# cvjena/ITAL

Measured on AMD Instinct MI355X. Metric: MI-scored candidates/sec per fetch_unlabelled(k) round, higher is better.
Workload: dtype f64; 1 GPU; USPS-shaped synthetic 9298x256, k=4, perfect user, full 2^t enumeration, fetch_unlabelled + update per step; n=9298, d=256, k=4, parallelism=candidate rows sharded over 1 GPU(s), 1 record all-gather per greedy step

## Files before the change

include/ital_hip.h:

```cpp
#ifndef ITAL_HIP_H
#define ITAL_HIP_H

#include <stdint.h>

#ifdef __cplusplus
extern "C" {
#endif

typedef struct ihipStream_t* hipStream_t;

#define ITAL_MAX_T 8
#define ITAL_REC_HEADER 10
#define ITAL_JUMP_BITS 48
#define ITAL_GENERIC_MAX_DIM 20
#define ITAL_GENERIC_MAX_REL 16
#define ITAL_GENERIC_MAX_CALLS (1 << 22)
#define ITAL_TOPK_MAX 4096
#define ITAL_ROUND_MAX_CAND (1 << 21)

const char* ital_version(void);
const char* ital_last_error(void);
int64_t ital_launch_count(void);


int ital_row_norms(const double* X, int64_t n, int ldx, double* xnorm, hipStream_t stream);

int ital_rbf_cols(const double* X, const double* xnorm, int64_t n, int ldx, const double* Xs, const double* sn,
                  int c, double var, double length_scale, double* out, int64_t ldo, hipStream_t stream);

int ital_cross_cov_cols(const double* X, const double* xnorm, int64_t n, int ldx, const double* Xs,
                        const double* sn, int c, const double* W, int ldw, const double* V, int64_t ldv, int m,
                        double var, double length_scale, double* out, int64_t ldo, hipStream_t stream);

int ital_chol_append(const double* XT, const double* XTn, int ldx, double* L, int ldl, double* alpha,
                     const double* ynew, int m, int c, double var, double length_scale, double noise, int* status,
                     hipStream_t stream);

typedef struct ital_label_batch {
    int c;
    int slot[16];
    double y[16];
} ital_label_batch;
int ital_stage_labelled(const double* rows, int ldx, ital_label_batch lb, double* XT_dst, double* XTn_dst, double* y_dst,
                        hipStream_t stream);

typedef struct ital_append_desc {
    const double* rows;
    int ldx;
    ital_label_batch lb;
    const double* X;
    const double* xnorm;
    int64_t n;
    double* XT;
    double* XTn;
    double* L;
    int ldl;
    double* alpha;
    double* ybuf;
    double* V;
    int64_t ldv;
    int m;
    double var, length_scale, noise;
    double* mu;
    double* s2;
    int* status;
} ital_append_desc;
int ital_gp_append(const ital_append_desc* a, hipStream_t stream);

int ital_whiten_append(const double* X, const double* xnorm, int64_t n, int ldx, const double* Xnew,
                       const double* snew, int c, const double* L21, int ldw, const double* L22,
                       const double* alpha_new, double* V, int64_t ldv, int m, double var, double length_scale,
                       double* mu, double* s2, hipStream_t stream);

int ital_predict(const double* Xt, int64_t nt, int ldx, const double* XT, const double* XTn, int m, const double* L,
                 int ldl, const double* alpha, double var, double length_scale, double* mean, double* pvar, double* xtn,
                 double* Vt, int64_t ldvt, int clamp, hipStream_t stream);

int ital_topk(const double* v, int64_t n, int64_t index_offset, int k, double* out_vals, int64_t* out_idx, void* work,
              hipStream_t stream);
int64_t ital_topk_workspace(void);

int ital_mvn_seed(int state[6]);
int ital_mvn_draws_per_call(int n);
int ital_mvn_advance(int state[6], int64_t n_draws);
int ital_mvn_round_seeds(int state[6], int64_t n_cand, int k, int seeds[][6]);
int ital_mvn_tables(int t, long long* jump, long long* jumppat, double* vk);
int ital_mvn_generic_tables(int nmax, long long* jump1, double* vk_all);

typedef struct ital_np_legacy_state {
    uint32_t key[624];
    int32_t pos;
    int32_t has_gauss;
    double gauss;
} ital_np_legacy_state;
int ital_np_legacy_normals(ital_np_legacy_state* st, int64_t n_skip, double* out, int64_t n_out, int threads);

typedef struct ital_batch {
    int kmax;
    int ldx;
    int ldw;
    int64_t* bidx;
    int64_t* bgpos;
    int32_t* bsort;
    double* bmu;
    double* sig;
    double* XB;
    double* XBn;
    double* VB;
} ital_batch;

typedef struct ital_score_desc {
    int t;
    int64_t n_cand;
    const int32_t* cand;
    const uint8_t* alive;
    const double* mu;
    const double* s2;
    const double* C;
    int64_t ldc;
    int64_t row_offset;
    int64_t pos_offset;
    const int64_t* gpos;
    ital_batch batch;
    double noise, eps;
    int label_mode;
    double* mi;
    int seed[6];
    const long long* jump;
    const long long* jumppat;
    const double* vk;
    int* status;
    double* work;
    int64_t work_doubles;
    void* ev_start;
    void* ev_stop;
    const double* sel_X;
    const double* sel_xnorm;
    int sel_ldx;
    const double* sel_V;
    int64_t sel_ldv;
    int sel_m, sel_ldw;
    int sel_rank;
    double* sel_record;
    int64_t* sel_ret;
    double* sel_parts;
    int64_t sel_parts_len;
    unsigned int* sel_counter;
} ital_score_desc;

int ital_score_step(const ital_score_desc* d, hipStream_t stream);

int64_t ital_score_workspace(int t, int64_t n_cand);

int ital_record_len(int ldx, int ldw, int kmax);
int64_t ital_round_workspace(int k, int64_t n_cand, int64_t cap_doubles);
int64_t ital_sel_parts_len(int k, int64_t n_cand, int64_t work_doubles);

typedef struct ital_round_desc {
    int k;
    ital_score_desc step;
    int seeds[ITAL_MAX_T + 1][6];
    const long long* jump[ITAL_MAX_T + 1];
    const long long* jumppat[ITAL_MAX_T + 1];
    const double* vk[ITAL_MAX_T + 1];
    void* ev_start[ITAL_MAX_T + 1];
    void* ev_stop[ITAL_MAX_T + 1];
    int64_t n_rows;
    double var, length_scale;
    double* mi_keep;
    int begin;
    const int32_t* cand_prev;
    int64_t n_prev;
    int world;
    double* records_all;
    void* nccl_comm;
    int (*exchange)(void* ctx, const double* record, double* records_all, int rec_len, hipStream_t stream);
    void* exchange_ctx;
} ital_round_desc;
int ital_fetch_round(const ital_round_desc* r, hipStream_t stream);

int ital_select_local(const double* mi, const int32_t* cand, const uint8_t* alive, int64_t n_cand, int64_t pos_offset,
                      const int64_t* gpos, int64_t row_offset, int rank, int mode, const double* mu, const double* s2,
                      const double* X, const double* xnorm, int ldx, const double* V, int64_t ldv, int m, int ldw,
                      const double* C, int64_t ldc, int nprev, int kmax, const int* status, double* work, double* record,
                      hipStream_t stream);

int ital_select_resolve(const double* records, int world, int rec_len, int rank, int mode, int slot,
                        ital_batch batch, uint8_t* alive, int64_t* ret, hipStream_t stream);

int ital_select_exchange(const double* record, double* records_all, int rec_len, void* nccl_comm, hipStream_t stream);

int ital_exchange_info(void* nccl_comm, int* world, int* rank, char* how, int how_len);

int ital_exchange_error(void* nccl_comm, int* async_error);

int ital_select_fused(const double* mi, const int32_t* cand, uint8_t* alive, int64_t n_cand, int64_t pos_offset,
                      const int64_t* gpos, int64_t row_offset, int rank, int mode, const double* mu, const double* s2,
                      const double* X, const double* xnorm, int ldx, const double* V, int64_t ldv, int m, int ldw,
                      const double* C, int64_t ldc, int nprev, int slot, ital_batch batch, const int* status,
                      double* record, int64_t* ret, hipStream_t stream);


int ital_gather_block(const int64_t* cand, int64_t nc, int64_t row0, int64_t n_rows, const double* X, const double* xnorm,
                      int ldx, const double* V, int64_t ldv, int m, const double* mu, const double* s2, double* Xc,
                      double* Vc, int64_t ldc, double* xnc, double* muc, double* s2c, hipStream_t stream);

int ital_cov_block(const double* Xa, const double* an, int64_t na, const double* Xb, const double* bn, int64_t nb,
                   int ldx, const double* Va, int64_t ldva, const double* Vb, int64_t ldvb, int m, double var,
                   double length_scale, double* out, int64_t ldo, hipStream_t stream);

int ital_cov_abs_rowsum(const double* Xa, const double* an, int64_t na, const double* Xb, const double* bn, int64_t nb,
                        int ldx, const double* Va, int64_t ldva, const double* Vb, int64_t ldvb, int m, double var,
                        double length_scale, double* work, int64_t work_len, int accumulate, double* out,
                        hipStream_t stream);

typedef struct ital_mcmi_desc {
    int t;
    int64_t n_i;
    int64_t pos_offset;
    int64_t n_all;
    const uint8_t* alive;
    const double* mu;
    const double* s2;
    const double* cov;
    int64_t ld_cov;
    const double* C;
    int64_t ldc;
    ital_batch batch;
    double noise, eps;
    double* ce;
    double* work;
    int64_t work_doubles;
} ital_mcmi_desc;

int ital_mcmi_score_step(const ital_mcmi_desc* d, hipStream_t stream);
int64_t ital_mcmi_workspace(int t, int64_t n_i);

typedef struct ital_mcmi_round_desc {
    int k;
    ital_mcmi_desc step;
    const double* Xc;
    const double* xnc;
    int ldx;
    const double* Vc;
    int64_t ldv;
    int m, ldw;
    double var, length_scale;
    const int32_t* pos;
    const int* status;
    double* record;
    int64_t* ret;
    int begin;
} ital_mcmi_round_desc;
int ital_mcmi_round(const ital_mcmi_round_desc* r, hipStream_t stream);

typedef struct ital_gscore_desc {
    int64_t n_cand;
    const int32_t* cand;
    const uint8_t* alive;
    const double* mu;
    const double* s2;
    const double* C;
    int64_t ldc;
    int64_t row_offset, pos_offset;
    const int64_t* gpos;
    int nE;
    const int64_t* E_idx;
    const int32_t* E_sort;
    const double* E_mu;
    const double* E_sig;
    int ldE;
    int n_picks;
    const int32_t* pick_pos;
    int subset_mode;
    int fb_mode;
    double label_prob, mistake_prob;
    int label_mode;
    double noise, eps;
    double clip_cov;
    int seed[6];
    const long long* jump1;
    const double* vk;
    int64_t draws_out;
    int64_t draws_in;
    int n_in;
    const int64_t* in_pos;
    int n_dead;
    const int64_t* dead_pos;
    int mc_rel;
    const uint32_t* rel_samples;
    int mc_fb;
    const uint32_t* fb_samples;
    const int64_t* draw_off;
    int64_t* draw_count;
    double* mi;
    int* status;
    double* work;
    int64_t work_doubles;
    unsigned long long* pair_count;
    int defer_join;
} ital_gscore_desc;

int ital_score_generic(const ital_gscore_desc* d, hipStream_t stream);
int64_t ital_score_generic_workspace(const ital_gscore_desc* d);
int ital_score_generic_join(hipStream_t stream);

typedef struct ital_ctx ital_ctx;
int ital_ctx_create(int64_t n_total, int d, double length_scale, double var, double noise, int capacity, int rank, int world,
                    void* nccl_comm, ital_ctx** out);
int ital_ctx_destroy(ital_ctx* ctx);
int ital_ctx_fit(ital_ctx* ctx, const double* rows, int on_device, hipStream_t stream);
int ital_ctx_update(ital_ctx* ctx, const int64_t* idx, const double* y, int c, hipStream_t stream);
int ital_ctx_fetch(ital_ctx* ctx, int k, int64_t* picks, hipStream_t stream);
int ital_ctx_predict_stored(ital_ctx* ctx, double* mean, double* variance, hipStream_t stream);
int64_t ital_ctx_local_rows(const ital_ctx* ctx, int64_t* row0);

#ifdef __cplusplus
}
#endif
#endif
```

ital_amd/_fast_round.py:

```python
import collections
import ctypes
import time

import numpy as np
import torch

from . import _lib, mvn_stream, sharding
from ._batch import (Scored, ensure_step_buffers, fill_score_desc, fill_score_select, lattice_label, lattice_tables)
from ._lib import check
from .gp import _ptr, _stream
from .retrieval_base import UnseenList

PREPARED, COMPACT, UPLOAD = "prepared", "compact", "upload"

DeviceList = collections.namedtuple("DeviceList", "buffers unseen version picks n_loc")


class Prepared(collections.namedtuple("Prepared", "desc slot k n n_loc m begin cur state_before state_after draws events sig")):
    __slots__ = ()

    def matches(self, k, n, m, stream_state, signature):
        return (self.k == k and self.n == n and self.m == m and self.state_before == tuple(stream_state)
                and self.sig == signature)

    def patch_share(self, n_loc, pos_offset):
        d = self.desc.step
        d.n_cand, d.pos_offset = n_loc, pos_offset
        return self._replace(n_loc=n_loc, events=[ev[:2] + (n_loc,) + ev[3:] for ev in self.events])


def plan_round(candidates, buffers, record, prepared, keep_scores, k, n, m, stream_state, signature):
    follows = (isinstance(candidates, UnseenList) and record is not None and record.buffers is buffers
               and record.unseen is candidates and record.version == candidates.version - 1
               and tuple(sorted(record.picks)) == candidates.last_removed)
    if not follows:
        return UPLOAD
    if prepared is not None and not keep_scores and prepared.matches(k, n, m, stream_state, signature):
        return PREPARED
    return COMPACT


class RoundBuffers(object):

    def __init__(self, learner, b):
        self.L, self.b = learner, b
        self.lists, self.cur = None, 0
        self.descs = None
        self.next = None
        self.exchange_cb = None
        self.exchange_exc = None
        self.device_list = None

    def invalidate(self):
        self.device_list = None

    def drop_prepared(self):
        if self.next is not None:
            for ev in self.next.events:
                self.L.event_pool += [ev[3], ev[4]]
            self.next = None

    def ensure(self, n_loc, k):
        L, b = self.L, self.b
        dev = L.gp.device
        grown = ensure_step_buffers(b, n_loc, L._sel_parts_doubles(k, n_loc), dev)
        if grown or self.lists is None or self.lists[0].numel() < n_loc:
            self.lists = [torch.empty(max(n_loc, 1), dtype=torch.int32, device=dev) for _ in range(2)]
            self.cur = 0
            self.descs = [_lib.ItalRoundDesc(), _lib.ItalRoundDesc()]
            self.drop_prepared()
            self.invalidate()

    def host_exchange(self):
        if self.exchange_cb is None:
            b, group = self.b, self.L.gp.group

            def exchange(ctx, record, records_all, rec_len, stream):
                try:
                    sharding.gather_records(b["rec"], b["rec_all"], group)
                    return 0
                except Exception as e:
                    self.exchange_exc = e
                    return -5
            self.exchange_cb = _lib.EXCHANGE_FN(exchange)
        return self.exchange_cb

    def signature(self, k):
        L, b = self.L, self.b
        gp = L.gp
        w = b.get("qmc_work")
        return (id(b), k, gp.cap, gp.ldv, gp.V.data_ptr(), gp.mu.data_ptr(), 0 if w is None else w.data_ptr(),
                float(L.noise), float(L.eps), float(L.var), float(L.length_scale), L.label_estimation, L.qmc_work_bytes,
                L.profile is not None, repr(L.profile_steps))

    def prepare(self, slot, k, n, m, begin, cur, state_before, *, n_prev=0, n_loc=None, pos_offset=0):
        L, b = self.L, self.b
        gp = L.gp
        r = self.descs[slot]
        d = r.step
        r.k, r.n_rows, r.var, r.length_scale = k, gp.n, float(L.var), float(L.length_scale)
        r.begin, r.cand_prev, r.n_prev = begin, (_ptr(self.lists[cur ^ 1]) if begin == 2 else None), (n_prev if begin == 2 else 0)
        n_loc = n if n_loc is None else n_loc
        fill_score_desc(d, gp, b, Scored(b["mi"], self.lists[cur], b["alive"], n_loc, pos_offset, None, gp.row0), L._user())
        r.world, r.records_all, r.nccl_comm, r.exchange = 0, None, None, _lib.EXCHANGE_FN(0)
        if gp.collective:
            kind, comm = L._round_transport()
            r.world, r.records_all = gp.world, _ptr(b["rec_all"])
            if kind == "nccl":
                r.nccl_comm = comm
            else:
                r.exchange = self.host_exchange()
        fill_score_select(d, gp, b, m, b["ret"])
        r.mi_keep = None
        work = None
        if k >= 3:
            work = L._qmc_workspace(b, k, n_loc)
            d.work, d.work_doubles = _ptr(work), work.numel()
        events = self._lattice_steps(r, k, n, n_loc, work)
        st6 = (ctypes.c_int * 6)(*state_before)
        check(_lib.lib().ital_mvn_round_seeds(st6, n, k, ctypes.byref(r.seeds)))
        draws = sum(mvn_stream.step_draws(t, n - (t - 1)) for t in range(3, k + 1))
        return Prepared(r, slot, k, n, n_loc, m, begin, cur, tuple(state_before), tuple(int(v) for v in st6), draws, events,
                        self.signature(k))

    def _lattice_steps(self, r, k, n, n_loc, work):
        L, b = self.L, self.b
        gp = L.gp
        events = []
        for t in range(1, k + 1):
            r.ev_start[t] = r.ev_stop[t] = None
            if t >= 3:
                r.jump[t], r.jumppat[t], r.vk[t] = [_ptr(x) for x in lattice_tables(b, t, gp.device)]
                if L.profile is not None and (L.profile_steps is None or t in L.profile_steps):
                    k0, k1 = L._event(), L._event()
                    r.ev_start[t], r.ev_stop[t] = k0.cuda_event, k1.cuda_event
                    events.append((lattice_label(work, t, n_loc), t,
                                   n - (t - 1) if not gp.collective else n_loc, k0, k1))
        return events


class FastRound(object):
    def __init__(self, learner, k, candidates):
        self.t_enter = time.perf_counter()
        self.L, self.k, self.candidates, self.gp = learner, k, candidates, learner.gp
        self.n = len(candidates)
        self.listed = isinstance(candidates, UnseenList)
        self.stream = mvn_stream.GLOBAL
        self.lo = self.n_loc = self.rb = self.p = self.keep = self.t_call = None

    def run(self):
        L = self.L
        self._share()
        self._buffers()
        self.p = p = self._descriptor()
        L.last_round = (p.begin, p.slot)
        self._keep_scores()
        saved_stream = (self.stream.state, self.stream.draws)
        self._stamp_call()
        self._call()
        self.stream.state, self.stream.draws = p.state_after, self.stream.draws + p.draws
        if L.profile is not None:
            L.profile += p.events
        self._prepare_next()
        ret, status = self._download()
        return self._finish(ret, status, saved_stream)

    def _share(self):
        gp, c = self.gp, self.candidates
        lo, hi = (c.count_below(gp.row0), c.count_below(gp.row1)) if gp.collective else (0, self.n)
        self.lo, self.n_loc = lo, hi - lo

    def _buffers(self):
        L = self.L
        b = L._buffers(self.k)
        if L._round_bufs is None:
            L._round_bufs = RoundBuffers(L, b)
        self.rb = L._round_bufs
        self.rb.ensure(self.n_loc, self.k)

    def _descriptor(self):
        L, gp, rb, k, n, n_loc = self.L, self.gp, self.rb, self.k, self.n, self.n_loc
        dl, p = rb.device_list, rb.next
        plan = plan_round(self.candidates, rb, dl, p, L.keep_scores, k, n, gp.m, self.stream.state,
                          rb.signature(k) if p is not None else None)
        rb.invalidate()
        if plan == PREPARED:
            rb.next = None
            rb.cur = p.cur
            return p.patch_share(n_loc, self.lo) if gp.collective else p
        rb.drop_prepared()
        if plan == COMPACT:
            begin, n_prev = 2, dl.n_loc
            rb.cur ^= 1
        else:
            begin, n_prev = 1, 0
            c = self.candidates
            share = c.in_rows(gp.row0, gp.row1) if self.listed else np.asarray(c, dtype=np.int64)
            rb.lists[rb.cur][:n_loc].copy_(torch.from_numpy((share - gp.row0).astype(np.int32)))
        return rb.prepare(0, k, n, gp.m, begin, rb.cur, self.stream.state, n_prev=n_prev, n_loc=n_loc, pos_offset=self.lo)

    def _keep_scores(self):
        if self.L.keep_scores:
            self.keep = torch.zeros((self.k, self.n_loc), dtype=torch.float64, device=self.gp.device)
            self.p.desc.mi_keep = _ptr(self.keep)

    def _stamp_call(self):
        hc = self.L.host_clock
        if hc is not None:
            self.t_call = t_call = time.perf_counter()
            if hc.get("t_download") is not None:
                hc["gap_s"] += t_call - hc["t_download"]
                hc["gaps"] += 1
                hc["prologue_s"] = hc.get("prologue_s", 0.0) + (t_call - self.t_enter)

    def _call(self):
        rb = self.rb
        rc = _lib.lib().ital_fetch_round(ctypes.byref(self.p.desc), _stream())
        if rc and rb.exchange_exc is not None:
            exc, rb.exchange_exc = rb.exchange_exc, None
            raise exc
        check(rc)

    def _prepare_next(self):
        L, gp, rb, p, k, n, n_loc = self.L, self.gp, self.rb, self.p, self.k, self.n, self.n_loc
        if n - k >= k and gp.m + k <= gp.cap and not L.keep_scores:
            rb.next = rb.prepare(p.slot ^ 1, k, n - k, gp.m + k, 2, rb.cur ^ 1, self.stream.state, n_prev=n_loc,
                                 n_loc=n_loc if gp.collective else n - k, pos_offset=self.lo)

    def _download(self):
        L, k, hc = self.L, self.k, self.L.host_clock
        if hc is not None:
            hc["enqueue_s"] += time.perf_counter() - self.t_call
        host = L._download(self.rb.b["ret"], "the picks of the round", L._step_estimate_s(k, self.n_loc)).tolist()
        if hc is not None:
            hc["t_download"] = time.perf_counter()
        keep = self.keep
        L.last_scores = [keep[t, :self.n_loc] for t in range(k)] if keep is not None else []
        return host[:k], host[self.rb.b["kmax"]]

    def _finish(self, ret, status, saved_stream):
        L, gp, c = self.L, self.gp, self.candidates
        if status & 8:
            raise RuntimeError("ital_amd: the candidate list kept on the device lost track of the host's (internal error)")
        if status & 6:
            gp.status.bitwise_and_(~6)
            self.stream.state, self.stream.draws = saved_stream
            return L._fetch_generic(self.k, c.array() if self.listed else c)
        if status:
            gp.check_status(status)
        ret = [int(i) for i in ret]
        L._last_batch = (self.rb.b, list(ret))
        if self.listed:
            self.rb.device_list = DeviceList(self.rb, c, c.version, ret, self.n_loc)
        return ret
```

ital_amd/_lib.py:

```python
import ctypes
import os

HERE = os.path.dirname(os.path.abspath(__file__))
LIB_PATH = os.environ.get("ITAL_HIP_LIB", os.path.join(HERE, "libital_hip.so"))

c_void_p, c_int, c_int64, c_double = ctypes.c_void_p, ctypes.c_int, ctypes.c_int64, ctypes.c_double

ITAL_MAX_T = 8
ITAL_REC_HEADER = 10
ITAL_JUMP_BITS = 48
ITAL_GENERIC_MAX_DIM = 20
ITAL_GENERIC_MAX_REL = 16
ITAL_GENERIC_MAX_CALLS = 1 << 22
ITAL_TOPK_MAX = 4096
ITAL_ROUND_MAX_CAND = 1 << 21


class ItalBatch(ctypes.Structure):
    _fields_ = [("kmax", c_int), ("ldx", c_int), ("ldw", c_int), ("bidx", c_void_p), ("bgpos", c_void_p),
                ("bsort", c_void_p), ("bmu", c_void_p), ("sig", c_void_p), ("XB", c_void_p), ("XBn", c_void_p),
                ("VB", c_void_p)]


class ItalLabelBatch(ctypes.Structure):
    _fields_ = [("c", c_int), ("slot", c_int * 16), ("y", c_double * 16)]


class ItalAppendDesc(ctypes.Structure):
    _fields_ = [("rows", c_void_p), ("ldx", c_int), ("lb", ItalLabelBatch), ("X", c_void_p), ("xnorm", c_void_p), ("n", c_int64),
                ("XT", c_void_p), ("XTn", c_void_p), ("L", c_void_p), ("ldl", c_int), ("alpha", c_void_p), ("ybuf", c_void_p),
                ("V", c_void_p), ("ldv", c_int64), ("m", c_int), ("var", c_double), ("length_scale", c_double),
                ("noise", c_double), ("mu", c_void_p), ("s2", c_void_p), ("status", c_void_p)]


class ItalScoreDesc(ctypes.Structure):
    _fields_ = [("t", c_int), ("n_cand", c_int64), ("cand", c_void_p), ("alive", c_void_p), ("mu", c_void_p),
                ("s2", c_void_p), ("C", c_void_p), ("ldc", c_int64), ("row_offset", c_int64),
                ("pos_offset", c_int64), ("gpos", c_void_p), ("batch", ItalBatch), ("noise", c_double), ("eps", c_double),
                ("label_mode", c_int), ("mi", c_void_p), ("seed", c_int * 6), ("jump", c_void_p), ("jumppat", c_void_p),
                ("vk", c_void_p), ("status", c_void_p), ("work", c_void_p), ("work_doubles", c_int64), ("ev_start", c_void_p),
                ("ev_stop", c_void_p), ("sel_X", c_void_p), ("sel_xnorm", c_void_p), ("sel_ldx", c_int), ("sel_V", c_void_p),
                ("sel_ldv", c_int64), ("sel_m", c_int), ("sel_ldw", c_int), ("sel_rank", c_int), ("sel_record", c_void_p),
                ("sel_ret", c_void_p), ("sel_parts", c_void_p), ("sel_parts_len", c_int64), ("sel_counter", c_void_p)]


EXCHANGE_FN = ctypes.CFUNCTYPE(c_int, c_void_p, c_void_p, c_void_p, c_int, c_void_p)


class ItalRoundDesc(ctypes.Structure):
    _fields_ = [("k", c_int), ("step", ItalScoreDesc), ("seeds", (c_int * 6) * (ITAL_MAX_T + 1)),
                ("jump", c_void_p * (ITAL_MAX_T + 1)), ("jumppat", c_void_p * (ITAL_MAX_T + 1)),
                ("vk", c_void_p * (ITAL_MAX_T + 1)), ("ev_start", c_void_p * (ITAL_MAX_T + 1)),
                ("ev_stop", c_void_p * (ITAL_MAX_T + 1)), ("n_rows", c_int64), ("var", c_double), ("length_scale", c_double),
                ("mi_keep", c_void_p), ("begin", c_int), ("cand_prev", c_void_p), ("n_prev", c_int64),
                ("world", c_int), ("records_all", c_void_p), ("nccl_comm", c_void_p), ("exchange", EXCHANGE_FN),
                ("exchange_ctx", c_void_p)]


class ItalGscoreDesc(ctypes.Structure):
    _fields_ = [("n_cand", c_int64), ("cand", c_void_p), ("alive", c_void_p), ("mu", c_void_p), ("s2", c_void_p),
                ("C", c_void_p), ("ldc", c_int64), ("row_offset", c_int64), ("pos_offset", c_int64), ("gpos", c_void_p),
                ("nE", c_int), ("E_idx", c_void_p), ("E_sort", c_void_p), ("E_mu", c_void_p), ("E_sig", c_void_p),
                ("ldE", c_int), ("n_picks", c_int), ("pick_pos", c_void_p), ("subset_mode", c_int), ("fb_mode", c_int),
                ("label_prob", c_double), ("mistake_prob", c_double), ("label_mode", c_int), ("noise", c_double),
                ("eps", c_double), ("clip_cov", c_double), ("seed", c_int * 6), ("jump1", c_void_p), ("vk", c_void_p),
                ("draws_out", c_int64), ("draws_in", c_int64), ("n_in", c_int), ("in_pos", c_void_p),
                ("n_dead", c_int), ("dead_pos", c_void_p), ("mc_rel", c_int), ("rel_samples", c_void_p),
                ("mc_fb", c_int), ("fb_samples", c_void_p), ("draw_off", c_void_p), ("draw_count", c_void_p), ("mi", c_void_p),
                ("status", c_void_p), ("work", c_void_p), ("work_doubles", c_int64), ("pair_count", c_void_p),
                ("defer_join", c_int)]


class ItalMcmiDesc(ctypes.Structure):
    _fields_ = [("t", c_int), ("n_i", c_int64), ("pos_offset", c_int64), ("n_all", c_int64), ("alive", c_void_p),
                ("mu", c_void_p), ("s2", c_void_p), ("cov", c_void_p), ("ld_cov", c_int64), ("C", c_void_p),
                ("ldc", c_int64), ("batch", ItalBatch), ("noise", c_double), ("eps", c_double), ("ce", c_void_p),
                ("work", c_void_p), ("work_doubles", c_int64)]


class ItalMcmiRoundDesc(ctypes.Structure):
    _fields_ = [("k", c_int), ("step", ItalMcmiDesc), ("Xc", c_void_p), ("xnc", c_void_p), ("ldx", c_int), ("Vc", c_void_p),
                ("ldv", c_int64), ("m", c_int), ("ldw", c_int), ("var", c_double), ("length_scale", c_double),
                ("pos", c_void_p), ("status", c_void_p), ("record", c_void_p), ("ret", c_void_p), ("begin", c_int)]


class ItalNpLegacyState(ctypes.Structure):
    _fields_ = [("key", ctypes.c_uint32 * 624), ("pos", ctypes.c_int32), ("has_gauss", ctypes.c_int32), ("gauss", c_double)]


SIGNATURES = {
    "ital_version": (ctypes.c_char_p, []),
    "ital_mvn_seed": (c_int, [ctypes.POINTER(c_int)]),
    "ital_mvn_draws_per_call": (c_int, [c_int]),
    "ital_mvn_advance": (c_int, [ctypes.POINTER(c_int), c_int64]),
    "ital_mvn_round_seeds": (c_int, [ctypes.POINTER(c_int), c_int64, c_int, c_void_p]),
    "ital_mvn_tables": (c_int, [c_int, c_void_p, c_void_p, c_void_p]),
    "ital_mvn_generic_tables": (c_int, [c_int, c_void_p, c_void_p]),
    "ital_np_legacy_normals": (c_int, [ctypes.POINTER(ItalNpLegacyState), c_int64, c_void_p, c_int64, c_int]),
    "ital_last_error": (ctypes.c_char_p, []),
    "ital_launch_count": (c_int64, []),
    "ital_row_norms": (c_int, [c_void_p, c_int64, c_int, c_void_p, c_void_p]),
    "ital_rbf_cols": (c_int, [c_void_p, c_void_p, c_int64, c_int, c_void_p, c_void_p, c_int, c_double, c_double,
                              c_void_p, c_int64, c_void_p]),
    "ital_cross_cov_cols": (c_int, [c_void_p, c_void_p, c_int64, c_int, c_void_p, c_void_p, c_int, c_void_p, c_int,
                                    c_void_p, c_int64, c_int, c_double, c_double, c_void_p, c_int64, c_void_p]),
    "ital_chol_append": (c_int, [c_void_p, c_void_p, c_int, c_void_p, c_int, c_void_p, c_void_p, c_int, c_int,
                                 c_double, c_double, c_double, c_void_p, c_void_p]),
    "ital_whiten_append": (c_int, [c_void_p, c_void_p, c_int64, c_int, c_void_p, c_void_p, c_int, c_void_p, c_int,
                                   c_void_p, c_void_p, c_void_p, c_int64, c_int, c_double, c_double, c_void_p,
                                   c_void_p, c_void_p]),
    "ital_stage_labelled": (c_int, [c_void_p, c_int, ItalLabelBatch, c_void_p, c_void_p, c_void_p, c_void_p]),
    "ital_gp_append": (c_int, [ctypes.POINTER(ItalAppendDesc), c_void_p]),
    "ital_predict": (c_int, [c_void_p, c_int64, c_int, c_void_p, c_void_p, c_int, c_void_p, c_int, c_void_p,
                             c_double, c_double, c_void_p, c_void_p, c_void_p, c_void_p, c_int64, c_int, c_void_p]),
    "ital_topk": (c_int, [c_void_p, c_int64, c_int64, c_int, c_void_p, c_void_p, c_void_p, c_void_p]),
    "ital_topk_workspace": (c_int64, []),
    "ital_score_step": (c_int, [ctypes.POINTER(ItalScoreDesc), c_void_p]),
    "ital_score_workspace": (c_int64, [c_int, c_int64]),
    "ital_fetch_round": (c_int, [ctypes.POINTER(ItalRoundDesc), c_void_p]),
    "ital_cov_block": (c_int, [c_void_p, c_void_p, c_int64, c_void_p, c_void_p, c_int64, c_int, c_void_p, c_int64,
                               c_void_p, c_int64, c_int, c_double, c_double, c_void_p, c_int64, c_void_p]),
    "ital_cov_abs_rowsum": (c_int, [c_void_p, c_void_p, c_int64, c_void_p, c_void_p, c_int64, c_int, c_void_p, c_int64,
                                    c_void_p, c_int64, c_int, c_double, c_double, c_void_p, c_int64, c_int, c_void_p,
                                    c_void_p]),
    "ital_mcmi_score_step": (c_int, [ctypes.POINTER(ItalMcmiDesc), c_void_p]),
    "ital_mcmi_workspace": (c_int64, [c_int, c_int64]),
    "ital_score_generic": (c_int, [ctypes.POINTER(ItalGscoreDesc), c_void_p]),
    "ital_score_generic_workspace": (c_int64, [ctypes.POINTER(ItalGscoreDesc)]),
    "ital_select_local": (c_int, [c_void_p, c_void_p, c_void_p, c_int64, c_int64, c_void_p, c_int64, c_int, c_int, c_void_p,
                                  c_void_p, c_void_p, c_void_p, c_int, c_void_p, c_int64, c_int, c_int, c_void_p,
                                  c_int64, c_int, c_int, c_void_p, c_void_p, c_void_p, c_void_p]),
    "ital_select_fused": (c_int, [c_void_p, c_void_p, c_void_p, c_int64, c_int64, c_void_p, c_int64, c_int, c_int, c_void_p,
                                  c_void_p, c_void_p, c_void_p, c_int, c_void_p, c_int64, c_int, c_int, c_void_p,
                                  c_int64, c_int, c_int, ItalBatch, c_void_p, c_void_p, c_void_p, c_void_p]),
    "ital_select_exchange": (c_int, [c_void_p, c_void_p, c_int, c_void_p, c_void_p]),
    "ital_exchange_info": (c_int, [c_void_p, c_void_p, c_void_p, ctypes.c_char_p, c_int]),
    "ital_exchange_error": (c_int, [c_void_p, c_void_p]),
    "ital_score_generic_join": (c_int, [c_void_p]),
    "ital_ctx_create": (c_int, [c_int64, c_int, c_double, c_double, c_double, c_int, c_int, c_int, c_void_p, c_void_p]),
    "ital_ctx_destroy": (c_int, [c_void_p]),
    "ital_ctx_fit": (c_int, [c_void_p, c_void_p, c_int, c_void_p]),
    "ital_ctx_update": (c_int, [c_void_p, c_void_p, c_void_p, c_int, c_void_p]),
    "ital_ctx_fetch": (c_int, [c_void_p, c_int, c_void_p, c_void_p]),
    "ital_ctx_predict_stored": (c_int, [c_void_p, c_void_p, c_void_p, c_void_p]),
    "ital_ctx_local_rows": (c_int64, [c_void_p, c_void_p]),
    "ital_record_len": (c_int, [c_int, c_int, c_int]),
    "ital_round_workspace": (c_int64, [c_int, c_int64, c_int64]),
    "ital_sel_parts_len": (c_int64, [c_int, c_int64, c_int64]),
    "ital_mcmi_round": (c_int, [ctypes.POINTER(ItalMcmiRoundDesc), c_void_p]),
    "ital_gather_block": (c_int, [c_void_p, c_int64, c_int64, c_int64, c_void_p, c_void_p, c_int, c_void_p, c_int64, c_int,
                                  c_void_p, c_void_p, c_void_p, c_void_p, c_int64, c_void_p, c_void_p, c_void_p, c_void_p]),
    "ital_select_resolve": (c_int, [c_void_p, c_int, c_int, c_int, c_int, c_int, ItalBatch, c_void_p, c_void_p,
                                    c_void_p]),
}


class ItalCtxModel(ctypes.Structure):
    _fields_ = [("label_prob", c_double), ("mistake_prob", c_double), ("label_estimation", c_int),
                ("monte_carlo_num_rel", c_int), ("monte_carlo_num_fb", c_int), ("clip_cov", c_double)]


CTX_SIGNATURES = {
    "ital_ctx_set_model": (c_int, [c_void_p, ctypes.POINTER(ItalCtxModel)]),
    "ital_ctx_fetch_list": (c_int, [c_void_p, c_int, c_void_p, c_int64, c_void_p, c_int, c_void_p, c_void_p]),
    "ital_ctx_mcmi_fetch": (c_int, [c_void_p, c_int, c_void_p, c_int64, c_void_p, c_void_p]),
    "ital_ctx_top_results": (c_int, [c_void_p, c_int, c_void_p, c_void_p]),
    "ital_ctx_predict": (c_int, [c_void_p, c_void_p, c_int64, c_void_p, c_void_p, c_void_p]),
    "ital_ctx_revoke": (c_int, [c_void_p, c_void_p, c_int, c_void_p]),
}


DENSE_SIGNATURES = {
    "ital_gram_rows": (c_int, [c_void_p, c_void_p, c_int, c_void_p, c_void_p, c_void_p, c_void_p, c_int, c_int, c_double,
                               c_double, c_double, c_void_p]),
    "ital_chol_batched": (c_int, [c_void_p, c_void_p, c_void_p, c_int, c_int, c_void_p, c_void_p, c_void_p]),
    "ital_chol_solve_batched": (c_int, [c_void_p, c_void_p, c_void_p, c_void_p, c_int, c_void_p, c_void_p]),
    "ital_kernel_matvec": (c_int, [c_void_p, c_void_p, c_int64, c_void_p, c_void_p, c_int64, c_int, c_void_p, c_int64, c_int,
                                   c_double, c_double, c_void_p, c_int64, c_void_p, c_int64, c_void_p]),
    "ital_kernel_matvec_workspace": (c_int64, [c_int64, c_int64]),
}


ADAPT_SIGNATURES = {
    "ital_chol_inv_diag": (c_int, [c_void_p, c_int, c_int64, c_void_p, c_void_p, c_int64, c_void_p, c_void_p]),
    "ital_chol_inv_diag_workspace": (c_int64, [c_int]),
    "ital_adapt_scores": (c_int, [c_void_p, c_void_p, c_void_p, c_int64, c_double, c_void_p, c_void_p, c_void_p]),
    "ital_adapt_error": (c_int, [c_void_p, c_int64, c_void_p, c_int, c_int64, c_void_p, c_void_p, c_double, c_void_p,
                                 c_void_p, c_void_p]),
}


class ItalRemoveDesc(ctypes.Structure):
    _fields_ = [("XT", c_void_p), ("XTn", c_void_p), ("ldx", c_int), ("L", c_void_p), ("ldl", c_int), ("alpha", c_void_p),
                ("V", c_void_p), ("ldv", c_int64), ("n", c_int64), ("mu", c_void_p), ("s2", c_void_p), ("m", c_int), ("p", c_int),
                ("work", c_void_p), ("work_doubles", c_int64), ("status", c_void_p)]


REVOKE_SIGNATURES = {
    "ital_gp_remove": (c_int, [ctypes.POINTER(ItalRemoveDesc), c_void_p]),
    "ital_gp_remove_workspace": (c_int64, [c_int]),
}


class ItalRewhitenDesc(ctypes.Structure):
    _fields_ = [("X", c_void_p), ("n_rows", c_int64), ("ldx", c_int), ("XT", c_void_p), ("XTn", c_void_p), ("L", c_void_p),
                ("ldl", c_int), ("alpha", c_void_p), ("m", c_int), ("var", c_double), ("length_scale", c_double),
                ("xnorm", c_void_p), ("V", c_void_p), ("ldv", c_int64), ("v_rows", c_int), ("mu", c_void_p), ("s2", c_void_p),
                ("chunk", c_int)]


REWHITEN_SIGNATURES = {
    "ital_whiten_rows": (c_int, [ctypes.POINTER(ItalRewhitenDesc), c_void_p]),
    "ital_whiten_rows_chunk": (c_int, []),
}


class ItalEvidenceDesc(ctypes.Structure):
    _fields_ = [("XT", c_void_p), ("XTn", c_void_p), ("ldx", c_int), ("y", c_void_p), ("m", c_int), ("params", c_void_p),
                ("G", c_int), ("K", c_void_p), ("ld", c_int64), ("scores", c_void_p), ("info", c_void_p),
                ("loo_mean", c_void_p), ("loo_var", c_void_p), ("ldm", c_int64), ("status", c_void_p), ("work", c_void_p),
                ("work_doubles", c_int64), ("ev", c_void_p)]


EVIDENCE_SIGNATURES = {
    "ital_gram_grid": (c_int, [c_void_p, c_void_p, c_int, c_int, c_void_p, c_int, c_void_p, c_int64, c_void_p]),
    "ital_chol_inv_diag_batched": (c_int, [c_void_p, c_void_p, c_int, c_int, c_void_p, c_void_p, c_int64, c_void_p, c_int64,
                                           c_void_p]),
    "ital_chol_inv_diag_batched_workspace": (c_int64, [c_int, c_int]),
    "ital_gp_evidence": (c_int, [ctypes.POINTER(ItalEvidenceDesc), c_void_p]),
    "ital_gp_evidence_workspace": (c_int64, [c_int, c_int]),
}


class ItalHipError(RuntimeError):
    pass


def load(path=LIB_PATH):
    if not os.path.exists(path):
        raise ImportError(
            f"{path} not found: build it with `python -m ital_amd.build` (hipcc, gfx950). "
            "ital_amd has no CPU fallback.")
    try:
        import torch
    except ImportError:
        pass
    lib = ctypes.CDLL(path)
    for name, (res, args) in list(SIGNATURES.items()) + list(CTX_SIGNATURES.items()) + list(DENSE_SIGNATURES.items()) + \
            list(ADAPT_SIGNATURES.items()) + list(REVOKE_SIGNATURES.items()) + list(REWHITEN_SIGNATURES.items()) + \
            list(EVIDENCE_SIGNATURES.items()):
        fn = getattr(lib, name)
        fn.restype = res
        fn.argtypes = args
    return lib


_lib = None


def lib():
    global _lib
    if _lib is None:
        _lib = load()
    return _lib


def check(rc):
    if rc != 0:
        raise ItalHipError(f"libital_hip: error {rc}: {lib().ital_last_error().decode()}")


def legacy_normals(n_skip, n_out, threads=1):
    import numpy as np
    n_skip, n_out = int(n_skip), int(n_out)
    state = np.random.get_state(legacy=True)
    if state[0] != "MT19937":
        if n_skip:
            np.random.standard_normal(n_skip)
        return np.random.standard_normal(n_out)
    st = ItalNpLegacyState()
    key = np.ascontiguousarray(state[1], dtype=np.uint32)
    ctypes.memmove(st.key, key.ctypes.data, 624 * 4)
    st.pos, st.has_gauss, st.gauss = int(state[2]), int(state[3]), float(state[4])
    out = np.empty(n_out, dtype=np.float64)
    check(lib().ital_np_legacy_normals(ctypes.byref(st), n_skip, out.ctypes.data, n_out, int(threads)))
    np.random.set_state(("MT19937", np.frombuffer(st.key, dtype=np.uint32).copy(), int(st.pos), int(st.has_gauss),
                         float(st.gauss)))
    return out
```

ital_amd/csrc/chol.hip:

```cpp
#include <hip/hip_runtime.h>
#include <stdint.h>

#include "device_math.h"
#include "ital_hip.h"
#include "ital_internal.h"

namespace ital {

__device__ __forceinline__ double readlane_f64(double v, int l) {
    return __hiloint2double(__builtin_amdgcn_readlane(__double2hiint(v), l), __builtin_amdgcn_readlane(__double2loint(v), l));
}

struct StageArgs {
    const double* rows;
    ital_label_batch lb;
    double* XT_w;
    double* XTn_w;
    double* y_w;
};

__global__ __launch_bounds__(1024) void chol_append_kernel(const double* XT, const double* XTn,
                                                           int ldx, double* __restrict__ L, int ldl,
                                                           double* __restrict__ alpha, const double* ynew,
                                                           int m, int c, double var, double s, double noise,
                                                           int* __restrict__ status, StageArgs sa) {
    __shared__ double S[16][17];
    __shared__ double tvec[16];
    __shared__ double Lb[64][65];
    const int lane = threadIdx.x & 63;
    const int j = threadIdx.x >> 6;
    const int g = m + j;
    double* Lg = L + (int64_t)g * ldl;
    if (sa.rows) {
        if (j < c) {
            const double* src = sa.rows + (int64_t)sa.lb.slot[j] * ldx;
            double* dst = sa.XT_w + (int64_t)j * ldx;
            double acc = 0;
            for (int k = lane; k < ldx; k += 64) {
                const double v = src[k];
                dst[k] = v;
                acc += v * v;
            }
            acc = wave_sum(acc);
            if (lane == 0) { sa.XTn_w[j] = acc; sa.y_w[j] = sa.lb.y[j]; }
        }
        __threadfence_block();
        __syncthreads();
    }
#ifdef ITAL_CHOL_TIMING
    long long tstamp[6];
    tstamp[0] = __builtin_readcyclecounter();
#define CHOL_STAMP(i) tstamp[i] = __builtin_readcyclecounter()
#else
#define CHOL_STAMP(i)
#endif
    {
        const int sub = threadIdx.x & 15;
        const int npair = (m + c) * c;
        for (int p0 = 0; p0 < npair; p0 += (int)blockDim.x >> 4) {
            const int pr = p0 + ((int)threadIdx.x >> 4);
            const bool live = pr < npair;
            const int jn = live ? pr % c : 0, r = live ? pr / c : 0;
            const int gn = m + jn;
            const bool need = live && r <= gn;
            double d0 = 0, d1 = 0;
            if (need) {
                const double* xa = XT + (int64_t)gn * ldx + 2 * sub;
                const double* xb = XT + (int64_t)r * ldx + 2 * sub;
                for (int k0 = 0; k0 < ldx; k0 += 256) {
                    double2 a[8], b[8];
#pragma unroll
                    for (int u = 0; u < 8; u++) {
                        const int k = k0 + 32 * u;
                        const bool in = k + 2 * sub < ldx;
                        a[u] = in ? *reinterpret_cast<const double2*>(xa + k) : double2{0, 0};
                        b[u] = in ? *reinterpret_cast<const double2*>(xb + k) : double2{0, 0};
                    }
#pragma unroll
                    for (int u = 0; u < 8; u++) {
                        d0 = fma(a[u].x, b[u].x, d0);
                        d1 = fma(a[u].y, b[u].y, d1);
                    }
                }
            }
            double dot = d0 + d1;
#pragma unroll
            for (int off = 1; off < 16; off <<= 1) dot += __shfl_xor(dot, off, 64);
            if (need && sub == 0) {
                double kv = var * exp((XTn[gn] + XTn[r] - 2 * dot) / s);
                if (r == gn) kv += noise;
                L[(int64_t)gn * ldl + r] = kv;
            }
        }
    }
    CHOL_STAMP(1);
    for (int r0 = 0; r0 < m; r0 += 64) {
        const int nb = m - r0 < 64 ? m - r0 : 64;
        __syncthreads();
        for (int idx = threadIdx.x; idx < nb * nb; idx += blockDim.x) {
            const int i = idx / nb, q = idx - i * nb;
            Lb[i][q] = L[(int64_t)(r0 + i) * ldl + r0 + q];
        }
        __syncthreads();
        if (j < c) {
            const bool in = lane < nb;
            double b = 0.0;
            if (in) {
                b = Lg[r0 + lane];
                const double* Li = L + (int64_t)(r0 + lane) * ldl;
                for (int q = 0; q < r0; q++) b = fma(-Li[q], Lg[q], b);
            }
            const double dinv = in ? 1.0 / Lb[lane][lane] : 1.0;
            double lq = Lb[lane][0];
            for (int q = 0; q < nb; q++) {
                const double lnext = Lb[lane][q + 1 < nb ? q + 1 : q];
                const double xq = readlane_f64(b * dinv, q);
                if (lane == q) b = xq;
                else if (lane > q && in) b = fma(-lq, xq, b);
                lq = lnext;
            }
            if (in) Lg[r0 + lane] = b;
            __builtin_amdgcn_fence(__ATOMIC_RELEASE, "workgroup");
            __builtin_amdgcn_wave_barrier();
            __builtin_amdgcn_fence(__ATOMIC_ACQUIRE, "workgroup");
        }
    }
    CHOL_STAMP(2);
    __threadfence_block();
    __syncthreads();
    if (j < c) {
        for (int q = 0; q <= j; q++) {
            const double* Lq = L + (int64_t)(m + q) * ldl;
            double acc = 0;
            for (int r = lane; r < m; r += 64) acc += Lg[r] * Lq[r];
            acc = wave_sum(acc);
            if (lane == 0) S[j][q] = Lg[m + q] - acc;
        }
        double acc = 0;
        for (int r = lane; r < m; r += 64) acc += Lg[r] * alpha[r];
        acc = wave_sum(acc);
        if (lane == 0) tvec[j] = ynew[j] - acc;
    }
    CHOL_STAMP(3);
    __syncthreads();
    if (j == 0) {
        const bool mine = lane < c;
        bool bad = false;
        for (int b = 0; b < c; b++) {
            const double dbb = S[b][b];
            if (!(dbb > 0)) bad = true;
            const double sq = sqrt(dbb);
            double lab = 0;
            if (mine && lane > b) {
                lab = S[lane][b] / sq;
                S[lane][b] = lab;
            }
            if (lane == b) S[b][b] = sq;
            __builtin_amdgcn_fence(__ATOMIC_RELEASE, "workgroup");
            __builtin_amdgcn_wave_barrier();
            __builtin_amdgcn_fence(__ATOMIC_ACQUIRE, "workgroup");
            if (mine && lane > b)
                for (int b2 = b + 1; b2 <= lane; b2++) S[lane][b2] -= lab * S[b2][b];
            __builtin_amdgcn_fence(__ATOMIC_RELEASE, "workgroup");
            __builtin_amdgcn_wave_barrier();
            __builtin_amdgcn_fence(__ATOMIC_ACQUIRE, "workgroup");
        }
        double tv = mine ? tvec[lane] : 0.0;
        const double dd = mine ? S[lane][lane] : 1.0;
        for (int q = 0; q < c; q++) {
            const double xq = readlane_f64(tv, q) / readlane_f64(dd, q);
            if (lane == q) tv = xq;
            else if (mine && lane > q) tv -= S[lane][q] * xq;
        }
        if (mine) {
            for (int b = 0; b < c; b++) L[(int64_t)(m + lane) * ldl + m + b] = b <= lane ? S[lane][b] : 0.0;
            alpha[m + lane] = tv;
        }
        if (bad && lane == 0) atomicOr(status, 1);
    }
#ifdef ITAL_CHOL_TIMING
    CHOL_STAMP(4);
    if (threadIdx.x == 0)
        for (int i = 0; i < 4; i++) alpha[ldl - 8 + i] = (double)(tstamp[i + 1] - tstamp[i]);
#endif
}

}

extern "C" int ital_chol_append(const double* XT, const double* XTn, int ldx, double* L, int ldl, double* alpha,
                                const double* ynew, int m, int c, double var, double length_scale, double noise,
                                int* status, hipStream_t stream) {
    if (c < 1 || c > 16) return ital_fail(-22, "ital_chol_append: c must be in 1..16");
    if (m < 0 || m + c > ldl) return ital_fail(-22, "ital_chol_append: factor capacity exceeded");
    ITAL_LAUNCH(ital::chol_append_kernel, dim3(1), dim3(1024), 0, stream, XT, XTn, ldx, L, ldl, alpha, ynew, m,
                       c, var, -2.0 * length_scale * length_scale, noise, status, ital::StageArgs{});
    return ital_check_launch("ital_chol_append");
}

extern "C" int ital_gp_append(const ital_append_desc* a, hipStream_t stream) {
    if (!a) return ital_fail(-22, "ital_gp_append: null descriptor");
    const int c = a->lb.c, m = a->m;
    if (c < 1 || c > 16) return ital_fail(-22, "ital_gp_append: 1..16 samples per call");
    if (m < 0 || m + c > a->ldl) return ital_fail(-22, "ital_gp_append: factor capacity exceeded");
    if (a->ldx % 16 != 0) return ital_fail(-22, "ital_gp_append: ldx must be a multiple of 16");
    ital::StageArgs sa = {a->rows, a->lb, a->XT + (int64_t)m * a->ldx, a->XTn + m, a->ybuf};
    ITAL_LAUNCH(ital::chol_append_kernel, dim3(1), dim3(1024), 0, stream, a->XT, a->XTn, a->ldx, a->L, a->ldl, a->alpha,
                a->ybuf, m, c, a->var, -2.0 * a->length_scale * a->length_scale, a->noise, a->status, sa);
    const int rc = ital_check_launch("ital_gp_append(chol)");
    if (rc) return rc;
    const double* L21 = a->L + (int64_t)m * a->ldl;
    return ital_whiten_append(a->X, a->xnorm, a->n, a->ldx, a->XT + (int64_t)m * a->ldx, a->XTn + m, c, L21, a->ldl, L21 + m,
                              a->alpha + m, a->V, a->ldv, m, a->var, a->length_scale, a->mu, a->s2, stream);
}
```

ital_amd/csrc/rbf.hip:

```cpp
#include <hip/hip_runtime.h>
#include <stdint.h>

#include "device_math.h"
#include "ital_hip.h"
#include "ital_internal.h"
#include "qmc_seed.h"

namespace ital {

typedef double d4 __attribute__((ext_vector_type(4)));

__global__ __launch_bounds__(256) void row_norms_kernel(const double* __restrict__ X, int64_t n, int ldx,
                                                        double* __restrict__ xnorm) {
    int64_t wave = ((int64_t)blockIdx.x * blockDim.x + threadIdx.x) >> 6;
    int lane = threadIdx.x & 63;
    int64_t nwaves = ((int64_t)gridDim.x * blockDim.x) >> 6;
    for (int64_t i = wave; i < n; i += nwaves) {
        const double* row = X + i * ldx;
        double acc = 0;
        for (int k = lane * 2; k < ldx; k += 128) {
            double2 v = *reinterpret_cast<const double2*>(row + k);
            acc += v.x * v.x + v.y * v.y;
        }
        acc = wave_sum(acc);
        if (lane == 0) xnorm[i] = acc;
    }
}

struct KcolsArgs {
    const double* X;
    const double* xnorm;
    int64_t n;
    int ldx;
    const double* Xs;
    const double* sn;
    int c;
    const double* W;
    int ldw;
    const double* V;
    int64_t ldv;
    int m;
    double var, s;
    int mode;
    double* out;
    int64_t ldo;
    const double* L22;
    const double* alpha_new;
    double* Vw;
    double* mu;
    double* s2;
};

enum { MODE_RAW = 0, MODE_WHITEN = 1 };
#ifndef ITAL_KCOLS_KU
#define ITAL_KCOLS_KU 4
#endif
constexpr int KU = ITAL_KCOLS_KU;

__device__ __forceinline__ void kcols_body(const KcolsArgs& a) {
    __shared__ double tile[4][16][17];
    const int lane = threadIdx.x & 63;
    const int wave = threadIdx.x >> 6;
    const int col = lane & 15;
    const int kg = lane >> 4;
    const int64_t i0 = ((int64_t)blockIdx.x * 4 + wave) * 16;
    if (i0 >= a.n) return;
    const int64_t irow = i0 + col;
    const bool row_ok = irow < a.n;
    const bool sel_ok = col < a.c;
    const double* xrow = a.X + (row_ok ? irow : 0) * a.ldx;
    const double* srow = a.Xs + (sel_ok ? col : 0) * (int64_t)a.ldx;

    d4 acc_dot = {0, 0, 0, 0};
    for (int k0 = 0; k0 < a.ldx; k0 += 16 * KU) {
        double2 b01[KU], b23[KU], a01[KU], a23[KU];
#pragma unroll
        for (int u = 0; u < KU; u++) {
            const int kk = k0 + 16 * u + 4 * kg;
            const bool in = k0 + 16 * u < a.ldx;
            b01[u] = b23[u] = a01[u] = a23[u] = double2{0, 0};
            if (in && row_ok) {
                b01[u] = *reinterpret_cast<const double2*>(xrow + kk);
                b23[u] = *reinterpret_cast<const double2*>(xrow + kk + 2);
            }
            if (in && sel_ok) {
                a01[u] = *reinterpret_cast<const double2*>(srow + kk);
                a23[u] = *reinterpret_cast<const double2*>(srow + kk + 2);
            }
        }
#pragma unroll
        for (int u = 0; u < KU; u++) {
            acc_dot = __builtin_amdgcn_mfma_f64_16x16x4f64(a01[u].x, b01[u].x, acc_dot, 0, 0, 0);
            acc_dot = __builtin_amdgcn_mfma_f64_16x16x4f64(a01[u].y, b01[u].y, acc_dot, 0, 0, 0);
            acc_dot = __builtin_amdgcn_mfma_f64_16x16x4f64(a23[u].x, b23[u].x, acc_dot, 0, 0, 0);
            acc_dot = __builtin_amdgcn_mfma_f64_16x16x4f64(a23[u].y, b23[u].y, acc_dot, 0, 0, 0);
        }
    }
    d4 acc_s = {0, 0, 0, 0};
    for (int r0 = 0; r0 < a.m; r0 += 16) {
        double av[4], bv[4];
#pragma unroll
        for (int u = 0; u < 4; u++) {
            const int r = r0 + 4 * u + kg;
            av[u] = bv[u] = 0;
            if (r < a.m) {
                if (sel_ok) av[u] = a.W[(int64_t)col * a.ldw + r];
                if (row_ok) bv[u] = a.V[(int64_t)r * a.ldv + irow];
            }
        }
#pragma unroll
        for (int u = 0; u < 4; u++) acc_s = __builtin_amdgcn_mfma_f64_16x16x4f64(av[u], bv[u], acc_s, 0, 0, 0);
    }
    const double xn = row_ok ? a.xnorm[irow] : 0.0;
    double R[4];
#pragma unroll
    for (int reg = 0; reg < 4; reg++) {
        const int j = kg + 4 * reg;
        double v = 0;
        if (j < a.c) {
            const double snj = a.sn[j];
            v = a.var * exp((snj + xn - 2 * acc_dot[reg]) / a.s) - acc_s[reg];
        }
        R[reg] = v;
    }
    if (a.mode == MODE_RAW) {
#pragma unroll
        for (int reg = 0; reg < 4; reg++) {
            const int j = kg + 4 * reg;
            if (j < a.c && row_ok) a.out[(int64_t)j * a.ldo + irow] = R[reg];
        }
        return;
    }
#pragma unroll
    for (int reg = 0; reg < 4; reg++) tile[wave][kg + 4 * reg][col] = R[reg];
    __builtin_amdgcn_fence(__ATOMIC_RELEASE, "wavefront");
    __builtin_amdgcn_wave_barrier();
    __builtin_amdgcn_fence(__ATOMIC_ACQUIRE, "wavefront");
    if (lane < 16 && row_ok) {
        double vn[16];
        double dvar = 0, dmu = 0;
#pragma unroll
        for (int j = 0; j < 16; j++) {
            if (j < a.c) {
                double acc = tile[wave][j][lane];
#pragma unroll
                for (int q = 0; q < j; q++) acc -= a.L22[j * a.ldw + q] * vn[q];
                vn[j] = acc / a.L22[j * a.ldw + j];
                dvar += vn[j] * vn[j];
                dmu += vn[j] * a.alpha_new[j];
                a.Vw[(int64_t)(a.m + j) * a.ldv + irow] = vn[j];
            } else {
                vn[j] = 0;
            }
        }
        a.s2[irow] -= dvar;
        a.mu[irow] += dmu;
    }
}

__global__ __launch_bounds__(256) void kcols_kernel(KcolsArgs a) { kcols_body(a); }

__global__ __launch_bounds__(256) void kcols_seed_kernel(KcolsArgs a, SeedArgs s, unsigned nk) {
    if (blockIdx.x >= nk) {
        qmc_seed_body(s, (int64_t)(blockIdx.x - nk) * 256 + threadIdx.x);
        return;
    }
    kcols_body(a);
}

__global__ __launch_bounds__(256) void predict_init_kernel(int64_t nt, double var, double* __restrict__ mean,
                                                           double* __restrict__ pvar) {
    const int64_t i = (int64_t)blockIdx.x * blockDim.x + threadIdx.x;
    if (i < nt) { mean[i] = 0.0; pvar[i] = var; }
}

__global__ __launch_bounds__(256) void clamp0_kernel(int64_t nt, double* __restrict__ pvar) {
    const int64_t i = (int64_t)blockIdx.x * blockDim.x + threadIdx.x;
    if (i < nt) pvar[i] = fmax(0.0, pvar[i]);
}

__global__ __launch_bounds__(64) void stage_labelled_kernel(const double* __restrict__ rows, int ldx, ital_label_batch lb,
                                                            double* __restrict__ XT_dst, double* __restrict__ XTn_dst,
                                                            double* __restrict__ y_dst) {
    const int j = blockIdx.x, lane = threadIdx.x;
    if (j >= lb.c) return;
    const double* src = rows + (int64_t)lb.slot[j] * ldx;
    double* dst = XT_dst + (int64_t)j * ldx;
    double acc = 0;
    for (int k = lane; k < ldx; k += 64) {
        const double v = src[k];
        dst[k] = v;
        acc += v * v;
    }
    acc = wave_sum(acc);
    if (lane == 0) { XTn_dst[j] = acc; y_dst[j] = lb.y[j]; }
}

}

using namespace ital;

extern "C" int ital_stage_labelled(const double* rows, int ldx, ital_label_batch lb, double* XT_dst, double* XTn_dst,
                                   double* y_dst, hipStream_t stream) {
    if (lb.c < 1 || lb.c > 16) return ital_fail(-22, "ital_stage_labelled: 1..16 samples per call");
    if (ldx % 16 != 0) return ital_fail(-22, "ital_stage_labelled: ldx must be a multiple of 16");
    ITAL_LAUNCH(stage_labelled_kernel, dim3(lb.c), dim3(64), 0, stream, rows, ldx, lb, XT_dst, XTn_dst, y_dst);
    return ital_check_launch("ital_stage_labelled");
}

extern "C" int ital_row_norms(const double* X, int64_t n, int ldx, double* xnorm, hipStream_t stream) {
    if (n <= 0) return 0;
    if (ldx % 16 != 0) return ital_fail(-22, "ital_row_norms: ldx must be a multiple of 16");
    int64_t blocks = (n + 3) / 4;
    if (blocks > 8192) blocks = 8192;
    ITAL_LAUNCH(row_norms_kernel, dim3((unsigned)blocks), dim3(256), 0, stream, X, n, ldx, xnorm);
    return ital_check_launch("ital_row_norms");
}

static int launch_kcols(KcolsArgs& a, hipStream_t stream, const char* who) {
    if (a.n <= 0) return 0;
    if (a.ldx % 16 != 0) return ital_fail(-22, "kcols: ldx must be a multiple of 16");
    if (a.c < 1 || a.c > 16) return ital_fail(-22, "kcols: c must be in 1..16");
    if (a.m < 0 || (a.m > 0 && (!a.W || !a.V))) return ital_fail(-22, "kcols: W/V missing");
    int64_t blocks = (a.n + 63) / 64;
    ITAL_LAUNCH(kcols_kernel, dim3((unsigned)blocks), dim3(256), 0, stream, a);
    return ital_check_launch(who);
}

extern "C" int ital_rbf_cols(const double* X, const double* xnorm, int64_t n, int ldx, const double* Xs,
                             const double* sn, int c, double var, double length_scale, double* out, int64_t ldo,
                             hipStream_t stream) {
    KcolsArgs a = {};
    a.X = X; a.xnorm = xnorm; a.n = n; a.ldx = ldx; a.Xs = Xs; a.sn = sn; a.c = c;
    a.m = 0; a.var = var; a.s = -2.0 * length_scale * length_scale; a.mode = MODE_RAW; a.out = out; a.ldo = ldo;
    return launch_kcols(a, stream, "ital_rbf_cols");
}

extern "C" int ital_cross_cov_cols(const double* X, const double* xnorm, int64_t n, int ldx, const double* Xs,
                                   const double* sn, int c, const double* W, int ldw, const double* V, int64_t ldv,
                                   int m, double var, double length_scale, double* out, int64_t ldo,
                                   hipStream_t stream) {
    KcolsArgs a = {};
    a.X = X; a.xnorm = xnorm; a.n = n; a.ldx = ldx; a.Xs = Xs; a.sn = sn; a.c = c;
    a.W = W; a.ldw = ldw; a.V = V; a.ldv = ldv; a.m = m;
    a.var = var; a.s = -2.0 * length_scale * length_scale; a.mode = MODE_RAW; a.out = out; a.ldo = ldo;
    return launch_kcols(a, stream, "ital_cross_cov_cols");
}

int ital_cross_cov_cols_seed(const double* X, const double* xnorm, int64_t n, int ldx, const double* Xs, const double* sn, int c,
                             const double* W, int ldw, const double* V, int64_t ldv, int m, double var, double length_scale,
                             double* out, int64_t ldo, const ital::SeedArgs& seed, hipStream_t stream) {
    KcolsArgs a = {};
    a.X = X; a.xnorm = xnorm; a.n = n; a.ldx = ldx; a.Xs = Xs; a.sn = sn; a.c = c;
    a.W = W; a.ldw = ldw; a.V = V; a.ldv = ldv; a.m = m;
    a.var = var; a.s = -2.0 * length_scale * length_scale; a.mode = MODE_RAW; a.out = out; a.ldo = ldo;
    if (a.n <= 0 || seed.slab_n <= 0) return ital_fail(-22, "ital_cross_cov_cols_seed: nothing to do");
    if (a.ldx % 16 != 0) return ital_fail(-22, "kcols: ldx must be a multiple of 16");
    if (a.c < 1 || a.c > 16) return ital_fail(-22, "kcols: c must be in 1..16");
    if (a.m < 0 || (a.m > 0 && (!a.W || !a.V))) return ital_fail(-22, "kcols: W/V missing");
    const int64_t nk = (a.n + 63) / 64, ns = (seed.slab_n + 255) / 256;
    ITAL_LAUNCH(kcols_seed_kernel, dim3((unsigned)(nk + ns)), dim3(256), 0, stream, a, seed, (unsigned)nk);
    return ital_check_launch("ital_cross_cov_cols_seed");
}

extern "C" int ital_whiten_append(const double* X, const double* xnorm, int64_t n, int ldx, const double* Xnew,
                                  const double* snew, int c, const double* L21, int ldw, const double* L22,
                                  const double* alpha_new, double* V, int64_t ldv, int m, double var,
                                  double length_scale, double* mu, double* s2, hipStream_t stream) {
    KcolsArgs a = {};
    a.X = X; a.xnorm = xnorm; a.n = n; a.ldx = ldx; a.Xs = Xnew; a.sn = snew; a.c = c;
    a.W = L21; a.ldw = ldw; a.V = V; a.Vw = V; a.ldv = ldv; a.m = m;
    a.var = var; a.s = -2.0 * length_scale * length_scale; a.mode = MODE_WHITEN;
    a.L22 = L22; a.alpha_new = alpha_new; a.mu = mu; a.s2 = s2;
    return launch_kcols(a, stream, "ital_whiten_append");
}

extern "C" int ital_predict(const double* Xt, int64_t nt, int ldx, const double* XT, const double* XTn, int m,
                            const double* L, int ldl, const double* alpha, double var, double length_scale,
                            double* mean, double* pvar, double* xtn, double* Vt, int64_t ldvt, int clamp,
                            hipStream_t stream) {
    if (nt <= 0) return 0;
    if (m <= 0) return ital_fail(-22, "ital_predict: GP is not fitted");
    if (!mean || !pvar || !xtn || !Vt) return ital_fail(-22, "ital_predict: mean / pvar / xtn / Vt must all be given");
    if (ldvt < nt) return ital_fail(-22, "ital_predict: ldvt smaller than the number of test points");
    int rc = ital_row_norms(Xt, nt, ldx, xtn, stream);
    if (rc) return rc;
    const unsigned blocks = (unsigned)((nt + 255) / 256);
    ITAL_LAUNCH(predict_init_kernel, dim3(blocks), dim3(256), 0, stream, nt, var, mean, pvar);
    for (int c0 = 0; c0 < m; c0 += 16) {
        const int c = m - c0 < 16 ? m - c0 : 16;
        rc = ital_whiten_append(Xt, xtn, nt, ldx, XT + (int64_t)c0 * ldx, XTn + c0, c, L + (int64_t)c0 * ldl, ldl,
                                L + (int64_t)c0 * ldl + c0, alpha + c0, Vt, ldvt, c0, var, length_scale, mean, pvar, stream);
        if (rc) return rc;
    }
    if (clamp) ITAL_LAUNCH(clamp0_kernel, dim3(blocks), dim3(256), 0, stream, nt, pvar);
    return ital_check_launch("ital_predict");
}
```

ital_amd/csrc/round.hip:

```cpp
#include <hip/hip_runtime.h>
#include <stdint.h>

#include "ital_hip.h"
#include "ital_internal.h"
#include "qmc_seed.h"

int ital_score_step_internal(const ital_score_desc* d, hipStream_t stream, bool seeds_ready, ital::SeedArgs* seeds_only);
int ital_cross_cov_cols_seed(const double* X, const double* xnorm, int64_t n, int ldx, const double* Xs, const double* sn, int c,
                             const double* W, int ldw, const double* V, int64_t ldv, int m, double var, double length_scale,
                             double* out, int64_t ldo, const ital::SeedArgs& seed, hipStream_t stream);

namespace ital {

__global__ __launch_bounds__(1024) void fetch_begin_kernel(int mode, const int32_t* __restrict__ cand_prev, int64_t n_prev,
                                                           int32_t* __restrict__ cand_new, uint8_t* __restrict__ alive,
                                                           int64_t n, int64_t* __restrict__ ret, int kmax,
                                                           int* __restrict__ status) {
    __shared__ int wave_tot[16];
    __shared__ int s_total;
    const int tid = threadIdx.x, lane = tid & 63, wave = tid >> 6;
    if (mode == 1) {
        const int64_t chunk = (n_prev + blockDim.x - 1) / blockDim.x;
        const int64_t lo = (int64_t)tid * chunk, hi = lo + chunk < n_prev ? lo + chunk : n_prev;
        int cnt = 0;
        for (int64_t p = lo; p < hi; p++) cnt += alive[p] != 0;
        int incl = cnt;
#pragma unroll
        for (int off = 1; off < 64; off <<= 1) {
            const int o = __shfl_up(incl, off, 64);
            if (lane >= off) incl += o;
        }
        if (lane == 63) wave_tot[wave] = incl;
        __syncthreads();
        int base = 0;
        for (int w = 0; w < wave; w++) base += wave_tot[w];
        if (tid == 0) {
            int tot = 0;
            for (int w = 0; w < (int)(blockDim.x >> 6); w++) tot += wave_tot[w];
            s_total = tot;
        }
        int64_t at = base + incl - cnt;
        for (int64_t p = lo; p < hi; p++)
            if (alive[p] != 0) cand_new[at++] = cand_prev[p];
        __syncthreads();
        if (tid == 0 && s_total != n) atomicOr(status, 8);
    }
    for (int64_t p = tid; p < n; p += blockDim.x) alive[p] = 1;
    if (tid == 0) ret[kmax] = 0;
}

constexpr int64_t COMPACT_TILE = 16384;
constexpr int64_t COMPACT_FROM = 1 << 16;

__device__ __forceinline__ unsigned tile_flags(const uint8_t* __restrict__ alive, int64_t at, int64_t n_prev) {
    unsigned m = 0;
    if (at + 16 <= n_prev) {
        const uint64_t* w = reinterpret_cast<const uint64_t*>(alive + at);
        const uint64_t lo = w[0], hi = w[1];
#pragma unroll
        for (int j = 0; j < 8; j++) {
            m |= (((lo >> (8 * j)) & 0xffull) != 0 ? 1u : 0u) << j;
            m |= (((hi >> (8 * j)) & 0xffull) != 0 ? 1u : 0u) << (8 + j);
        }
    } else {
        for (int j = 0; j < 16 && at + j < n_prev; j++) m |= (alive[at + j] != 0 ? 1u : 0u) << j;
    }
    return m;
}

__device__ __forceinline__ int block_sum_1024(int v, int* s_wave) {
    const int lane = threadIdx.x & 63, wave = threadIdx.x >> 6;
#pragma unroll
    for (int off = 32; off > 0; off >>= 1) v += __shfl_xor(v, off, 64);
    if (lane == 0) s_wave[wave] = v;
    __syncthreads();
    int tot = 0;
    for (int w = 0; w < 16; w++) tot += s_wave[w];
    __syncthreads();
    return tot;
}

__global__ __launch_bounds__(1024) void compact_count_kernel(const uint8_t* __restrict__ alive, int64_t n_prev, int* __restrict__ counts) {
    __shared__ int s_wave[16];
    const int64_t at = (int64_t)blockIdx.x * COMPACT_TILE + (int64_t)threadIdx.x * 16;
    const int cnt = at < n_prev ? __popc(tile_flags(alive, at, n_prev)) : 0;
    const int tot = block_sum_1024(cnt, s_wave);
    if (threadIdx.x == 0) counts[blockIdx.x] = tot;
}

__global__ __launch_bounds__(1024) void compact_scatter_kernel(const int32_t* __restrict__ cand_prev, const uint8_t* __restrict__ alive,
                                                               int64_t n_prev, int32_t* __restrict__ cand_new,
                                                               const int* __restrict__ counts) {
    __shared__ int s_wave[16];
    const int lane = threadIdx.x & 63, wave = threadIdx.x >> 6;
    int64_t base = 0;
    for (int b = 0; b < (int)blockIdx.x; b++) base += counts[b];
    const int64_t at = (int64_t)blockIdx.x * COMPACT_TILE + (int64_t)threadIdx.x * 16;
    const unsigned m = at < n_prev ? tile_flags(alive, at, n_prev) : 0u;
    const int cnt = __popc(m);
    int incl = cnt;
#pragma unroll
    for (int off = 1; off < 64; off <<= 1) {
        const int o = __shfl_up(incl, off, 64);
        if (lane >= off) incl += o;
    }
    if (lane == 63) s_wave[wave] = incl;
    __syncthreads();
    int before = incl - cnt;
    for (int w = 0; w < wave; w++) before += s_wave[w];
    int64_t out = base + before;
    for (unsigned mm = m; mm; mm &= mm - 1) cand_new[out++] = cand_prev[at + __builtin_ctz(mm)];
}

__global__ __launch_bounds__(1024) void compact_rearm_kernel(uint8_t* __restrict__ alive, int64_t n, int64_t* __restrict__ ret, int kmax,
                                                             int* __restrict__ status, const int* __restrict__ counts, int ntiles) {
    const int64_t stride = (int64_t)gridDim.x * blockDim.x;
    for (int64_t p = (int64_t)blockIdx.x * blockDim.x + threadIdx.x; p < n; p += stride) alive[p] = 1;
    if (blockIdx.x == 0 && threadIdx.x == 0) {
        int64_t tot = 0;
        for (int b = 0; b < ntiles; b++) tot += counts[b];
        if (tot != n) atomicOr(status, 8);
        ret[kmax] = 0;
    }
}

}

using namespace ital;

extern "C" int ital_fetch_round(const ital_round_desc* r, hipStream_t stream) {
    if (!r) return ital_fail(-22, "ital_fetch_round: null descriptor");
    const ital_score_desc& tpl = r->step;
    if (r->k < 1 || r->k > ITAL_MAX_T || r->k > tpl.batch.kmax) return ital_fail(-22, "ital_fetch_round: k outside 1..min(ITAL_MAX_T, kmax)");
    const bool ranks = r->world > 0;
    if (ranks && (!r->records_all || (!r->nccl_comm && !r->exchange)))
        return ital_fail(-22, "ital_fetch_round: several ranks need records_all and a transport (nccl_comm or exchange)");
    if (ranks ? tpl.n_cand < 1 : tpl.n_cand < r->k)
        return ital_fail(-22, "ital_fetch_round: fewer candidates than greedy steps (several ranks: none on this rank)");
    if (tpl.n_cand > ITAL_ROUND_MAX_CAND) return ital_fail(-22, "ital_fetch_round: more than ITAL_ROUND_MAX_CAND candidates (use the per-step entry points)");
    if (!tpl.sel_record || !tpl.sel_ret) return ital_fail(-22, "ital_fetch_round: the round selects inside the scorer: sel_* missing");
    if (r->begin < 0 || r->begin > 2) return ital_fail(-22, "ital_fetch_round: begin must be 0, 1 or 2");
    if (r->begin == 2 && (!r->cand_prev || r->n_prev < tpl.n_cand || r->n_prev > ITAL_ROUND_MAX_CAND || r->cand_prev == tpl.cand))
        return ital_fail(-22, "ital_fetch_round: begin = 2 needs the previous list in a buffer of its own");
    if (r->begin == 2 && r->n_prev >= COMPACT_FROM) {
        const unsigned ntiles = (unsigned)((r->n_prev + COMPACT_TILE - 1) / COMPACT_TILE);
        if (!tpl.sel_parts || tpl.sel_parts_len * 2 < (int64_t)ntiles + 1)
            return ital_fail(-22, "ital_fetch_round: step.sel_parts too small for the tile counts of the list upkeep (ital_sel_parts_len)");
        int* counts = reinterpret_cast<int*>(tpl.sel_parts);
        uint8_t* alive = const_cast<uint8_t*>(tpl.alive);
        ITAL_LAUNCH(compact_count_kernel, dim3(ntiles), dim3(1024), 0, stream, alive, r->n_prev, counts);
        ITAL_LAUNCH(compact_scatter_kernel, dim3(ntiles), dim3(1024), 0, stream, r->cand_prev, alive, r->n_prev,
                    const_cast<int32_t*>(tpl.cand), counts);
        ITAL_LAUNCH(compact_rearm_kernel, dim3(ntiles), dim3(1024), 0, stream, alive, tpl.n_cand, tpl.sel_ret, tpl.batch.kmax,
                    tpl.status, counts, (int)ntiles);
        const int rc = ital_check_launch("ital_fetch_round(begin, tiles)");
        if (rc) return rc;
    } else if (r->begin) {
        ITAL_LAUNCH(fetch_begin_kernel, dim3(1), dim3(1024), 0, stream, r->begin - 1, r->cand_prev, r->n_prev,
                    const_cast<int32_t*>(tpl.cand), const_cast<uint8_t*>(tpl.alive), tpl.n_cand, tpl.sel_ret, tpl.batch.kmax,
                    tpl.status);
        const int rc = ital_check_launch("ital_fetch_round(begin)");
        if (rc) return rc;
    }
    auto step_desc = [&](int t) {
        ital_score_desc d = tpl;
        d.t = t;
        if (r->mi_keep) d.mi = r->mi_keep + (int64_t)(t - 1) * tpl.n_cand;
        if (t >= 3) {
            d.jump = r->jump[t];
            d.jumppat = r->jumppat[t];
            d.vk = r->vk[t];
            for (int j = 0; j < 6; j++) d.seed[j] = r->seeds[t][j];
        }
        d.ev_start = r->ev_start[t];
        d.ev_stop = r->ev_stop[t];
        if (ranks) d.sel_ret = nullptr;
        return d;
    };
    const int rec_len = ITAL_REC_HEADER + tpl.sel_ldx + tpl.sel_ldw + tpl.batch.kmax;
    bool seeds_ready = false;
    for (int t = 1; t <= r->k; t++) {
        const ital_score_desc d = step_desc(t);
        int rc = ital_score_step_internal(&d, stream, seeds_ready, nullptr);
        if (rc) return rc;
        seeds_ready = false;
        if (ranks) {
            rc = r->exchange ? r->exchange(r->exchange_ctx, tpl.sel_record, r->records_all, rec_len, stream)
                             : ital_select_exchange(tpl.sel_record, r->records_all, rec_len, r->nccl_comm, stream);
            if (rc) return r->exchange ? ital_fail(rc, "ital_fetch_round: the host's exchange failed") : rc;
            rc = ital_select_resolve(r->records_all, r->world, rec_len, tpl.sel_rank, 0, t - 1, tpl.batch,
                                     const_cast<uint8_t*>(tpl.alive), tpl.sel_ret, stream);
            if (rc) return rc;
        }
        if (t < r->k) {
            const int slot = t - 1;
            const double* xb = tpl.batch.XB + (int64_t)slot * tpl.batch.ldx;
            const double* vb = tpl.batch.VB + (int64_t)slot * tpl.batch.ldw;
            double* col = const_cast<double*>(tpl.C) + (int64_t)slot * tpl.ldc;
            SeedArgs seed;
            const ital_score_desc nx = step_desc(t + 1);
            if (ital_score_step_internal(&nx, stream, false, &seed) == 0) {
                rc = ital_cross_cov_cols_seed(tpl.sel_X, tpl.sel_xnorm, r->n_rows, tpl.sel_ldx, xb, tpl.batch.XBn + slot, 1, vb,
                                              tpl.batch.ldw, tpl.sel_V, tpl.sel_ldv, tpl.sel_m, r->var, r->length_scale, col,
                                              tpl.ldc, seed, stream);
                seeds_ready = true;
            } else {
                rc = ital_cross_cov_cols(tpl.sel_X, tpl.sel_xnorm, r->n_rows, tpl.sel_ldx, xb, tpl.batch.XBn + slot, 1, vb,
                                         tpl.batch.ldw, tpl.sel_V, tpl.sel_ldv, tpl.sel_m, r->var, r->length_scale, col, tpl.ldc,
                                         stream);
            }
            if (rc) return rc;
        }
    }
    return 0;
}

extern "C" int ital_mcmi_round(const ital_mcmi_round_desc* r, hipStream_t stream) {
    if (!r) return ital_fail(-22, "ital_mcmi_round: null descriptor");
    const ital_mcmi_desc& tpl = r->step;
    if (r->k < 1 || r->k > ITAL_MAX_T || r->k > tpl.batch.kmax) return ital_fail(-22, "ital_mcmi_round: k outside 1..min(ITAL_MAX_T, kmax)");
    if (tpl.pos_offset != 0 || tpl.n_i != tpl.n_all) return ital_fail(-22, "ital_mcmi_round: one rank scores the whole block (pos_offset 0, n_i == n_all)");
    if (tpl.n_all < r->k) return ital_fail(-22, "ital_mcmi_round: fewer candidates than greedy steps");
    if (tpl.n_all > (1 << 18)) return ital_fail(-22, "ital_mcmi_round: more than 2^18 candidates (use the per-step entry points)");
    if (!r->Xc || !r->xnc || !r->pos || !r->record || !r->ret || !tpl.alive || !tpl.cov || (r->m > 0 && !r->Vc))
        return ital_fail(-22, "ital_mcmi_round: null argument");
    uint8_t* alive = const_cast<uint8_t*>(tpl.alive);
    int rc;
    if (r->begin) {
        ITAL_LAUNCH(fetch_begin_kernel, dim3(1), dim3(1024), 0, stream, 0, nullptr, (int64_t)0, nullptr, alive, tpl.n_i, r->ret,
                    tpl.batch.kmax, const_cast<int*>(r->status));
        if ((rc = ital_check_launch("ital_mcmi_round(begin)"))) return rc;
    }
    rc = ital_cov_block(r->Xc, r->xnc, tpl.n_i, r->Xc, r->xnc, tpl.n_all, r->ldx, r->Vc, r->ldv, r->Vc, r->ldv, r->m, r->var,
                        r->length_scale, const_cast<double*>(tpl.cov), tpl.ld_cov, stream);
    if (rc) return rc;
    for (int t = 1; t <= r->k; t++) {
        ital_mcmi_desc d = tpl;
        d.t = t;
        if ((rc = ital_mcmi_score_step(&d, stream))) return rc;
        rc = ital_select_fused(tpl.ce, r->pos, alive, tpl.n_i, 0, nullptr, 0, 0, 1, tpl.mu, tpl.s2, r->Xc, r->xnc, r->ldx, r->Vc,
                               r->ldv, r->m, r->ldw, tpl.C, tpl.ldc, t - 1, t - 1, tpl.batch, r->status, r->record, r->ret, stream);
        if (rc) return rc;
        if (t < r->k) {
            const int slot = t - 1;
            rc = ital_cross_cov_cols(r->Xc, r->xnc, tpl.n_all, r->ldx, tpl.batch.XB + (int64_t)slot * tpl.batch.ldx,
                                     tpl.batch.XBn + slot, 1, tpl.batch.VB + (int64_t)slot * tpl.batch.ldw, tpl.batch.ldw, r->Vc,
                                     r->ldv, r->m, r->var, r->length_scale, const_cast<double*>(tpl.C) + (int64_t)slot * tpl.ldc,
                                     tpl.ldc, stream);
            if (rc) return rc;
        }
    }
    return 0;
}
```

ital_amd/gp.py:

```python
import ctypes
import os
import time

import numpy as np
import torch

from . import _lib, sharding
from ._lib import check


def _pad16(v):
    return (int(v) + 15) // 16 * 16


def _ptr(t):
    return 0 if t is None else t.data_ptr()


def _stream():
    return torch.cuda.current_stream().cuda_stream


def appends_after_remove(appends, p):
    out = list(appends)
    at = 0
    for g, c in enumerate(out):
        if at <= p < at + abs(c):
            if c < 0:
                raise ValueError("labelled position %d is a query" % p)
            out[g] = c - 1
            return out
        at += abs(c)
    raise ValueError("labelled position %d outside the %d labelled samples" % (p, at))


class GaussianProcess(object):

    def __init__(self, data, length_scale, var=1.0, noise=1e-6, pdist=None, *, device=None, rank=0, world=1,
                 group=None, capacity=None):
        if pdist is not None:
            raise NotImplementedError("pre-computed distances are a dense-kernel feature of the reference (gp.py:116-128)")
        if not torch.cuda.is_available():
            raise RuntimeError("ital_amd.GaussianProcess needs a HIP device (no CPU fallback)")
        self._lib = _lib.lib()
        self.device = torch.device(device if device is not None else "cuda:0")
        self.rank, self.world, self.group = int(rank), int(world), group
        self.collective = self.world > 1 or (group is not None and os.environ.get("ITAL_FORCE_COLLECTIVES") == "1")
        local = None
        if isinstance(data, sharding.ShardedRows):
            local = data
        else:
            data = np.asarray(data, dtype=np.float64)
        if data.ndim != 2:
            raise ValueError("data must be an n-by-d array")
        self.n_total, self.d = data.shape
        self.row0, self.row1 = sharding.row_range(self.n_total, self.world, self.rank)
        if local is not None and (local.row0, local.row1) != (self.row0, self.row1):
            raise ValueError("ShardedRows holds rows [%d, %d), this rank owns [%d, %d)"
                             % (local.row0, local.row1, self.row0, self.row1))
        self.n = self.row1 - self.row0
        self.ldx = _pad16(self.d)
        self.ldv = _pad16(max(self.n, 1))
        self.length_scale = length_scale
        self.length_scale_sq = length_scale * length_scale
        self.var = var
        self.noise = noise
        self.X_host = data
        with torch.cuda.device(self.device):
            Xp = torch.zeros((max(self.n, 1), self.ldx), dtype=torch.float64, device=self.device)
            if self.n:
                rows = local.local if local is not None else data[self.row0:self.row1]
                Xp[: self.n, : self.d] = torch.from_numpy(np.ascontiguousarray(rows)).to(self.device)
            self.Xd = Xp
            self.xnorm = torch.empty(max(self.n, 1), dtype=torch.float64, device=self.device)
            check(self._lib.ital_row_norms(_ptr(self.Xd), self.n, self.ldx, _ptr(self.xnorm), _stream()))
            self.status = torch.zeros(1, dtype=torch.int32, device=self.device)
            self._gather_bufs = {}
            if capacity is None:
                capacity = int(min(256, max(64, (2 << 30) // (8 * self.ldv))))
            self._alloc(capacity)
        self.reset()

    def _alloc(self, cap):
        cap = _pad16(cap)
        dev = self.device
        old = getattr(self, "cap", 0)
        V = torch.zeros((cap, self.ldv), dtype=torch.float64, device=dev)
        L = torch.zeros((cap, cap), dtype=torch.float64, device=dev)
        alpha = torch.zeros(cap, dtype=torch.float64, device=dev)
        XT = torch.zeros((cap, self.ldx), dtype=torch.float64, device=dev)
        XTn = torch.zeros(cap, dtype=torch.float64, device=dev)
        if old:
            V[:old] = self.V
            L[:old, :old] = self.L
            alpha[:old] = self.alpha
            XT[:old] = self.XT
            XTn[:old] = self.XTn
        self.V, self.L, self.alpha, self.XT, self.XTn, self.cap = V, L, alpha, XT, XTn, cap

    @property
    def X(self):
        return self.X_host

    @property
    def K_all(self):
        raise AttributeError("the dense N x N kernel matrix is never formed by ital_amd (reference gp.py:128 is "
                             "replaced by column streaming); use rbf_cols()")

    def _factor(self):
        return self.L[: self.m, : self.m].cpu().numpy()

    @property
    def K(self):
        if self.m == 0:
            return None
        f = self._factor()
        return f @ f.T

    @property
    def K_inv(self):
        if self.m == 0:
            return None
        fi = np.linalg.inv(self._factor())
        return fi.T @ fi

    @property
    def w(self):
        if self.m == 0:
            return None
        import scipy.linalg
        return scipy.linalg.solve_triangular(self._factor(), self.alpha[: self.m].cpu().numpy(), lower=True, trans="T")

    def kernel(self, a, b=None):
        if b is None:
            if self.m == 0:
                raise RuntimeError("the GP has not been fitted")
            a, b = self.XT[: self.m, : self.d].cpu().numpy(), a
        a = np.atleast_2d(np.asarray(a, dtype=np.float64))
        b = np.atleast_2d(np.asarray(b, dtype=np.float64))
        dev = self.device
        A = torch.zeros((len(a), self.ldx), dtype=torch.float64, device=dev)
        B = torch.zeros((len(b), self.ldx), dtype=torch.float64, device=dev)
        A[:, : self.d] = torch.from_numpy(np.ascontiguousarray(a)).to(dev)
        B[:, : self.d] = torch.from_numpy(np.ascontiguousarray(b)).to(dev)
        an = torch.empty(len(a), dtype=torch.float64, device=dev)
        bn = torch.empty(len(b), dtype=torch.float64, device=dev)
        out = torch.empty((len(a), _pad16(len(b))), dtype=torch.float64, device=dev)
        st = _stream()
        check(self._lib.ital_row_norms(_ptr(A), len(a), self.ldx, _ptr(an), st))
        check(self._lib.ital_row_norms(_ptr(B), len(b), self.ldx, _ptr(bn), st))
        check(self._lib.ital_cov_block(_ptr(A), _ptr(an), len(a), _ptr(B), _ptr(bn), len(b), self.ldx, 0, 0, 0, 0, 0,
                                       float(self.var), float(self.length_scale), _ptr(out), out.shape[1], st))
        return out[:, : len(b)].cpu().numpy()

    def reset(self):
        self.ind = []
        self.y = None
        self.m = 0
        self.appends = []
        self.mu = torch.zeros(max(self.n, 1), dtype=torch.float64, device=self.device)
        self.s2 = torch.full((max(self.n, 1),), float(self.var), dtype=torch.float64, device=self.device)
        self.mu_all = torch.zeros(self.n_total, dtype=torch.float64, device=self.device) if self.collective else self.mu[: self.n]
        self._mean_host = None
        self.status.zero_()

    def fit(self, ind, y):
        self.reset()
        return self.update(ind, y)

    def update(self, ind, y, row_cache=None):
        ind = [int(i) for i in ind]
        y = np.asarray(y, dtype=np.float64).reshape(-1)
        if len(ind) != len(y):
            raise ValueError("ind and y differ in length")
        if len(ind) == 0:
            return self
        hc = getattr(self, "host_clock", None)
        t0 = time.perf_counter() if hc is not None else 0.0
        if row_cache is not None and all(i in row_cache[1] for i in ind):
            if len(ind) <= 16:
                self._append_staged(row_cache[0], [row_cache[1][i] for i in ind], y)
            else:
                slots = torch.as_tensor([row_cache[1][i] for i in ind], dtype=torch.int64, device=self.device)
                self._append(row_cache[0].index_select(0, slots), y)
        else:
            self._append(self._gather_rows(ind), y)
        self.ind += ind
        self.y = y.copy() if self.y is None else np.concatenate((self.y, y))
        self.appends.append(len(ind))
        t1 = time.perf_counter() if hc is not None else 0.0
        self._replicate_mean()
        if hc is not None:
            hc["append_s"] = hc.get("append_s", 0.0) + (t1 - t0)
            hc["means_s"] = hc.get("means_s", 0.0) + (time.perf_counter() - t1)
        return self

    def update_points(self, points, y, ind=None):
        pts = np.atleast_2d(np.asarray(points, dtype=np.float64))
        y = np.asarray(y, dtype=np.float64).reshape(-1)
        rows = torch.zeros((len(pts), self.ldx), dtype=torch.float64, device=self.device)
        rows[:, : self.d] = torch.from_numpy(np.ascontiguousarray(pts)).to(self.device)
        self._append(rows, y)
        self.ind += list(ind) if ind is not None else list(range(self.n_total + self.m - len(y), self.n_total + self.m))
        self.y = y.copy() if self.y is None else np.concatenate((self.y, y))
        self.appends.append(-len(y))
        self._replicate_mean()
        return self

    def _owned(self, ind):
        idx = np.asarray([int(i) for i in ind], dtype=np.int64)
        own = (idx >= self.row0) & (idx < self.row1)
        loc = np.where(own, idx - self.row0, 0)
        return (torch.from_numpy(own.astype(np.float64)).to(self.device),
                torch.from_numpy(loc).to(self.device), bool(own.any()))

    def _gather_rows(self, ind):
        if not self.collective:
            idx = torch.as_tensor(ind, dtype=torch.int64, device=self.device)
            return self.Xd.index_select(0, idx)
        mask, loc, any_own = self._owned(ind)
        if any_own:
            rows = self.Xd.index_select(0, loc) * mask[:, None]
        else:
            rows = torch.zeros((len(ind), self.ldx), dtype=torch.float64, device=self.device)
        sharding.all_reduce_sum(rows, self.group)
        return rows

    def gather_columns(self, mat, ind):
        mask, loc, any_own = self._owned(ind)
        if any_own:
            out = mat.index_select(1, loc) * mask[None, :]
        else:
            out = torch.zeros((mat.shape[0], len(loc)), dtype=torch.float64, device=self.device)
        if self.collective:
            sharding.all_reduce_sum(out, self.group)
        return out

    def _append_staged(self, matrix, slots, y):
        c = len(slots)
        if self.m + c > self.cap:
            self._alloc(max(2 * self.cap, self.m + c))
        if getattr(self, "_ybuf", None) is None:
            self._ybuf = torch.empty(16, dtype=torch.float64, device=self.device)
        d = getattr(self, "_append_desc", None)
        key = (self.V.data_ptr(), self.mu.data_ptr(), self.cap)
        if d is None or d[0] != key:
            a = _lib.ItalAppendDesc()
            a.ldx, a.X, a.xnorm, a.n = self.ldx, _ptr(self.Xd), _ptr(self.xnorm), self.n
            a.XT, a.XTn, a.L, a.ldl, a.alpha, a.ybuf = _ptr(self.XT), _ptr(self.XTn), _ptr(self.L), self.cap, _ptr(self.alpha), \
                _ptr(self._ybuf)
            a.V, a.ldv, a.mu, a.s2, a.status = _ptr(self.V), self.ldv, _ptr(self.mu), _ptr(self.s2), _ptr(self.status)
            self._append_desc = d = (key, a)
        a = d[1]
        a.rows, a.m = _ptr(matrix), self.m
        a.var, a.length_scale, a.noise = float(self.var), float(self.length_scale), float(self.noise)
        a.lb.c = c
        for j in range(c):
            a.lb.slot[j] = int(slots[j])
            a.lb.y[j] = float(y[j])
        check(self._lib.ital_gp_append(ctypes.byref(a), _stream()))
        self.m += c

    def _append(self, rows, y):
        lib, st = self._lib, _stream()
        c_total = rows.shape[0]
        if self.m + c_total > self.cap:
            self._alloc(max(2 * self.cap, self.m + c_total))
        yd = torch.from_numpy(np.ascontiguousarray(y)).to(self.device)
        for c0 in range(0, c_total, 16):
            c = min(16, c_total - c0)
            m = self.m
            self.XT[m:m + c] = rows[c0:c0 + c]
            check(lib.ital_row_norms(_ptr(self.XT[m:m + c]), c, self.ldx, _ptr(self.XTn[m:m + c]), st))
            check(lib.ital_chol_append(_ptr(self.XT), _ptr(self.XTn), self.ldx, _ptr(self.L), self.cap, _ptr(self.alpha),
                                       _ptr(yd[c0:c0 + c]), m, c, float(self.var), float(self.length_scale),
                                       float(self.noise), _ptr(self.status), st))
            L21 = self.L[m:]
            check(lib.ital_whiten_append(_ptr(self.Xd), _ptr(self.xnorm), self.n, self.ldx, _ptr(self.XT[m:m + c]),
                                         _ptr(self.XTn[m:m + c]), c, _ptr(L21), self.cap,
                                         L21.data_ptr() + 8 * m, _ptr(self.alpha[m:m + c]), _ptr(self.V), self.ldv, m,
                                         float(self.var), float(self.length_scale), _ptr(self.mu), _ptr(self.s2), st))
            self.m += c

    def remove(self, ind):
        ind = [int(i) for i in ind]
        if not ind:
            return self
        if len(set(ind)) != len(ind):
            raise ValueError("a sample is named twice")
        pos_of = {i: p for p, i in enumerate(self.ind)}
        for i in ind:
            if i >= self.n_total:
                raise ValueError("%d is a query row: queries cannot be removed" % i)
            if i not in pos_of:
                raise ValueError("sample %d has no label" % i)
        lib, st = self._lib, _stream()
        need = int(lib.ital_gp_remove_workspace(self.cap))
        work = getattr(self, "_remove_work", None)
        if work is None or work.numel() < need:
            self._remove_work = work = torch.empty(need, dtype=torch.float64, device=self.device)
        r = _lib.ItalRemoveDesc()
        r.XT, r.XTn, r.ldx, r.L, r.ldl, r.alpha = _ptr(self.XT), _ptr(self.XTn), self.ldx, _ptr(self.L), self.cap, _ptr(self.alpha)
        r.V, r.ldv, r.n, r.mu, r.s2 = _ptr(self.V), self.ldv, self.n, _ptr(self.mu), _ptr(self.s2)
        r.work, r.work_doubles, r.status = _ptr(work), work.numel(), _ptr(self.status)
        for p in sorted((pos_of[i] for i in ind), reverse=True):
            r.m, r.p = self.m, p
            check(lib.ital_gp_remove(ctypes.byref(r), st))
            self.appends = appends_after_remove(self.appends, p)
            del self.ind[p]
            self.y = np.delete(self.y, p)
            self.m -= 1
        if self.m == 0:
            self.reset()
        self._replicate_mean()
        return self

    def _whiten_rows(self, row_start, n_rows):
        r = _lib.ItalRewhitenDesc()
        r.X, r.n_rows, r.ldx = self.Xd.data_ptr() + 8 * row_start * self.ldx, n_rows, self.ldx
        r.XT, r.XTn, r.L, r.ldl, r.alpha, r.m = _ptr(self.XT), _ptr(self.XTn), _ptr(self.L), self.cap, _ptr(self.alpha), self.m
        r.var, r.length_scale = float(self.var), float(self.length_scale)
        r.xnorm, r.V, r.ldv, r.v_rows = self.xnorm.data_ptr() + 8 * row_start, self.V.data_ptr() + 8 * row_start, self.ldv, self.cap
        r.mu, r.s2, r.chunk = self.mu.data_ptr() + 8 * row_start, self.s2.data_ptr() + 8 * row_start, 0
        check(self._lib.ital_whiten_rows(ctypes.byref(r), _stream()))

    def extend(self, rows):
        rows = np.asarray(rows, dtype=np.float64)
        if rows.size == 0:
            return self
        if rows.ndim != 2 or rows.shape[1] != self.d:
            raise ValueError("rows must be a k-by-%d array" % self.d)
        if self.world > 1 or not isinstance(self.X_host, np.ndarray):
            raise NotImplementedError("row sharding cannot grow yet: extend() needs all rows on one rank")
        k, n_old, m, dev = len(rows), self.n, self.m, self.device
        n_new = n_old + k
        ldv = _pad16(n_new)
        with torch.cuda.device(dev):
            Xd = torch.zeros((n_new, self.ldx), dtype=torch.float64, device=dev)
            Xd[:n_old] = self.Xd[:n_old]
            Xd[n_old:, : self.d] = torch.from_numpy(np.ascontiguousarray(rows)).to(dev)
            xnorm = torch.empty(n_new, dtype=torch.float64, device=dev)
            mu = torch.empty(n_new, dtype=torch.float64, device=dev)
            s2 = torch.empty(n_new, dtype=torch.float64, device=dev)
            V = torch.zeros((self.cap, ldv), dtype=torch.float64, device=dev)
            xnorm[:n_old], mu[:n_old], s2[:n_old] = self.xnorm[:n_old], self.mu[:n_old], self.s2[:n_old]
            if m and n_old:
                V[:m, :n_old] = self.V[:m, :n_old]
            self.Xd, self.xnorm, self.mu, self.s2, self.V = Xd, xnorm, mu, s2, V
            self.n, self.ldv = n_new, ldv
            self.ind = [i + k if i >= self.n_total else i for i in self.ind]
            self.n_total += k
            self.row1 = self.row0 + n_new
            self.X_host = np.concatenate((self.X_host, rows))
            self._append_desc = None
            self._gather_bufs = {}
            self._whiten_rows(n_old, k)
            self._replicate_mean()
        return self

    def set_params(self, length_scale=None, var=None, noise=None):
        ls = float(self.length_scale if length_scale is None else length_scale)
        var = float(self.var if var is None else var)
        noise = float(self.noise if noise is None else noise)
        if not (ls > 0 and var > 0):
            raise ValueError("length_scale and var must be positive")
        with torch.cuda.device(self.device):
            if self.m == 0:
                self.s2.fill_(var)
            else:
                lib, st, m = self._lib, _stream(), self.m
                L = torch.zeros((self.cap, self.cap), dtype=torch.float64, device=self.device)
                alpha = torch.zeros(self.cap, dtype=torch.float64, device=self.device)
                status = torch.zeros(1, dtype=torch.int32, device=self.device)
                yd = torch.from_numpy(np.ascontiguousarray(self.y, dtype=np.float64)).to(self.device)
                for c0 in range(0, m, 16):
                    c = min(16, m - c0)
                    check(lib.ital_chol_append(_ptr(self.XT), _ptr(self.XTn), self.ldx, _ptr(L), self.cap, _ptr(alpha),
                                               _ptr(yd[c0:c0 + c]), c0, c, var, ls, noise, _ptr(status), st))
                self.check_status(int(status.item()))
                self.L, self.alpha = L, alpha
                self._append_desc = None
            self.length_scale, self.length_scale_sq, self.var, self.noise = ls, ls * ls, var, noise
            if self.m:
                self._whiten_rows(0, self.n)
                self._replicate_mean()
        return self

    def evidence_chunk(self, max_bytes=1 << 30):
        m = self.m
        per = 8 * (m * m + int(self._lib.ital_gp_evidence_workspace(m, 1)) + 2 * m + 4)
        if per > max_bytes:
            raise MemoryError("one candidate at m = %d takes %d bytes, more than max_bytes = %d" % (m, per, max_bytes))
        return int(min(max_bytes // per, 65535))

    def evidence(self, params_list, *, max_bytes=1 << 30, events=None):
        if self.m == 0:
            raise RuntimeError("the GP has not been fitted")
        prm = np.empty((len(params_list), 3), dtype=np.float64)
        for g, p in enumerate(params_list):
            unknown = set(p) - {"length_scale", "var", "noise"}
            if unknown:
                raise TypeError("unexpected GP parameters: %s" % ", ".join(sorted(unknown)))
            prm[g] = (float(p.get("length_scale", self.length_scale)), float(p.get("var", self.var)),
                      float(p.get("noise", self.noise)))
            if not (prm[g, 0] > 0 and prm[g, 1] > 0):
                raise ValueError("length_scale and var must be positive")
        G, m, lib, dev = len(prm), self.m, self._lib, self.device
        out = dict(lml=np.empty(G), loo_logp=np.empty(G), loo_mse=np.empty(G), ok=np.zeros(G, dtype=bool),
                   loo_mean=np.empty((G, m)), loo_var=np.empty((G, m)))
        if G == 0:
            return out
        chunk = min(G, self.evidence_chunk(max_bytes))
        with torch.cuda.device(dev):
            yd = torch.from_numpy(np.ascontiguousarray(self.y, dtype=np.float64)).to(dev)
            pd = torch.from_numpy(prm).to(dev)
            K = torch.empty(chunk * m * m, dtype=torch.float64, device=dev)
            need = int(lib.ital_gp_evidence_workspace(m, chunk))
            work = torch.empty(need, dtype=torch.float64, device=dev)
            scores = torch.empty((chunk, 3), dtype=torch.float64, device=dev)
            info = torch.empty(chunk, dtype=torch.int32, device=dev)
            lm = torch.empty((chunk, m), dtype=torch.float64, device=dev)
            lv = torch.empty((chunk, m), dtype=torch.float64, device=dev)
            status = torch.zeros(1, dtype=torch.int32, device=dev)
            d = _lib.ItalEvidenceDesc()
            d.XT, d.XTn, d.ldx, d.y, d.m = _ptr(self.XT), _ptr(self.XTn), self.ldx, _ptr(yd), m
            d.K, d.ld, d.scores, d.info, d.loo_mean, d.loo_var, d.ldm = _ptr(K), m, _ptr(scores), _ptr(info), _ptr(lm), _ptr(lv), m
            d.status, d.work, d.work_doubles = _ptr(status), _ptr(work), need
            for g0 in range(0, G, chunk):
                c = min(chunk, G - g0)
                d.params, d.G = pd.data_ptr() + 24 * g0, c
                ev = None
                if events is not None and g0 + c == G:
                    ev = (ctypes.c_void_p * 6)(*[e.cuda_event for e in events])
                d.ev = ctypes.addressof(ev) if ev is not None else None
                check(lib.ital_gp_evidence(ctypes.byref(d), _stream()))
                sc = scores[:c].cpu().numpy()
                out["lml"][g0:g0 + c], out["loo_logp"][g0:g0 + c], out["loo_mse"][g0:g0 + c] = sc[:, 0], sc[:, 1], sc[:, 2]
                out["ok"][g0:g0 + c] = info[:c].cpu().numpy() == 0
                out["loo_mean"][g0:g0 + c] = lm[:c].cpu().numpy()
                out["loo_var"][g0:g0 + c] = lv[:c].cpu().numpy()
        return out

    def check_status(self, status=None):
        s = int(self.status.item()) if status is None else int(status)
        if s & 1:
            raise np.linalg.LinAlgError("kernel matrix of the labelled samples is not positive definite "
                                        "(the reference would warn at gp.py:31)")
        if s & 2:
            raise np.linalg.LinAlgError("singular conditional covariance in the orthant integrator "
                                        "(duplicate samples in the batch?)")

    def _full(self, t):
        return self._full_device(t).cpu().numpy()

    def _full_device(self, t, keep=None):
        loc = t[: self.n]
        if not self.collective:
            return loc
        pad = (self.n_total + self.world - 1) // self.world
        bufs = self._gather_bufs.get(keep) if keep else None
        if bufs is None:
            bufs = (torch.zeros(pad, dtype=loc.dtype, device=self.device),
                    torch.empty((self.world, pad), dtype=loc.dtype, device=self.device))
            if keep:
                self._gather_bufs[keep] = bufs
        send, recv = bufs
        if self.n == pad and loc.is_contiguous():
            send = loc
        else:
            send[: self.n] = loc
        sharding.gather_records(send, recv, self.group)
        if pad * self.world == self.n_total:
            return recv.view(-1)
        parts = []
        for r in range(self.world):
            a, b = sharding.row_range(self.n_total, self.world, r)
            parts.append(recv[r, : b - a])
        return torch.cat(parts)

    def _replicate_mean(self):
        self.mu_all = self._full_device(self.mu, keep="mu")
        self._mean_host = None

    def mean_host(self):
        if self._mean_host is None:
            self._mean_host = self.mu_all.cpu().numpy()
        return self._mean_host

    def topk_mean(self, k):
        k = int(k)
        n = self.n_total
        if not (1 <= k <= min(_lib.ITAL_TOPK_MAX, n)):
            raise ValueError("k outside 1..min(%d, number of samples)" % _lib.ITAL_TOPK_MAX)
        if getattr(self, "_topk_work", None) is None:
            self._topk_work = torch.empty(int(self._lib.ital_topk_workspace()), dtype=torch.uint8, device=self.device)
        vals = torch.empty(k, dtype=torch.float64, device=self.device)
        idx = torch.empty(k, dtype=torch.int64, device=self.device)
        check(self._lib.ital_topk(_ptr(self.mu_all), n, 0, k, _ptr(vals), _ptr(idx), _ptr(self._topk_work), _stream()))
        return idx.cpu().numpy()

    def predict_stored(self, ind=None, cov_mode=None):
        if self.m == 0:
            raise RuntimeError("the GP has not been fitted: call fit()/update() first "
                               "(the reference fails with an AttributeError at gp.py:222)")
        mean = self.mean_host()
        if ind is not None:
            ind = np.asarray(ind, dtype=np.int64)
            mean = mean[ind]
        if cov_mode is None:
            return mean
        if cov_mode == "diag":
            var = np.maximum(0, self._full(self.s2))
            return mean, (var if ind is None else var[ind])
        if cov_mode == "full":
            if ind is None:
                raise ValueError("full covariance of all samples is an N x N matrix; pass `ind`")
            return mean, self._cov_full(ind)
        raise ValueError("cov_mode must be None, 'diag' or 'full'")

    def _cov_full(self, ind):
        ind = [int(i) for i in ind]
        ns = len(ind)
        rows = self._gather_rows(ind)
        norms = torch.empty(ns, dtype=torch.float64, device=self.device)
        check(self._lib.ital_row_norms(_ptr(rows), ns, self.ldx, _ptr(norms), _stream()))
        lds = _pad16(ns)
        Vs = torch.zeros((max(self.m, 1), lds), dtype=torch.float64, device=self.device)
        Vs[: self.m, :ns] = self.gather_columns(self.V[: max(self.m, 1)], ind)[: self.m]
        out = torch.empty((ns, lds), dtype=torch.float64, device=self.device)
        check(self._lib.ital_cov_block(_ptr(rows), _ptr(norms), ns, _ptr(rows), _ptr(norms), ns, self.ldx, _ptr(Vs), lds,
                                       _ptr(Vs), lds, self.m, float(self.var), float(self.length_scale), _ptr(out), lds,
                                       _stream()))
        return out[:, :ns].cpu().numpy()

    def updated_prediction(self, ind, y, pred_ind, cov_mode=None):
        ind = [int(i) for i in ind]
        pred = [int(i) for i in pred_ind]
        y = np.asarray(y, dtype=np.float64).reshape(-1)
        mean, cov = self.predict_stored(pred + ind, cov_mode="full")
        n = len(pred)
        s_ff = cov[n:, n:] + self.noise * np.eye(len(ind))
        s_pf = cov[:n, n:]
        sol = np.linalg.solve(s_ff, np.column_stack((y - mean[n:], s_pf.T)))
        new_mean = mean[:n] + s_pf @ sol[:, 0]
        if cov_mode is None:
            return new_mean
        new_cov = cov[:n, :n] - s_pf @ sol[:, 1:]
        if cov_mode == "full":
            return new_mean, new_cov
        if cov_mode == "diag":
            return new_mean, np.maximum(0, np.diag(new_cov))
        raise ValueError("cov_mode must be None, 'diag' or 'full'")

    def rbf_cols(self, ind):
        rows = self._gather_rows([int(i) for i in ind])
        norms = torch.empty(len(ind), dtype=torch.float64, device=self.device)
        check(self._lib.ital_row_norms(_ptr(rows), len(ind), self.ldx, _ptr(norms), _stream()))
        out = torch.empty((len(ind), self.ldv), dtype=torch.float64, device=self.device)
        for c0 in range(0, len(ind), 16):
            c = min(16, len(ind) - c0)
            check(self._lib.ital_rbf_cols(_ptr(self.Xd), _ptr(self.xnorm), self.n, self.ldx, _ptr(rows[c0:c0 + c]),
                                          _ptr(norms[c0:c0 + c]), c, float(self.var), float(self.length_scale),
                                          _ptr(out[c0:c0 + c]), self.ldv, _stream()))
        return out[:, : self.n]

    def predict(self, X, cov_mode=None):
        if self.m == 0:
            raise RuntimeError("the GP has not been fitted")
        if cov_mode not in (None, "diag", "full"):
            raise ValueError("cov_mode must be None, 'diag' or 'full'")
        X = np.atleast_2d(np.asarray(X, dtype=np.float64))
        nt = X.shape[0]
        dev = self.device
        Xt = torch.zeros((nt, self.ldx), dtype=torch.float64, device=dev)
        Xt[:, : self.d] = torch.from_numpy(np.ascontiguousarray(X)).to(dev)
        ldvt = _pad16(nt)
        mean = torch.empty(nt, dtype=torch.float64, device=dev)
        pvar = torch.empty(nt, dtype=torch.float64, device=dev)
        xtn = torch.empty(nt, dtype=torch.float64, device=dev)
        Vt = torch.empty((self.m, ldvt), dtype=torch.float64, device=dev)
        check(self._lib.ital_predict(_ptr(Xt), nt, self.ldx, _ptr(self.XT), _ptr(self.XTn), self.m, _ptr(self.L), self.cap,
                                     _ptr(self.alpha), float(self.var), float(self.length_scale), _ptr(mean), _ptr(pvar),
                                     _ptr(xtn), _ptr(Vt), ldvt, 1, _stream()))
        if cov_mode == "diag":
            return mean.cpu().numpy(), pvar.cpu().numpy()
        if cov_mode == "full":
            cov = torch.empty((nt, ldvt), dtype=torch.float64, device=dev)
            check(self._lib.ital_cov_block(_ptr(Xt), _ptr(xtn), nt, _ptr(Xt), _ptr(xtn), nt, self.ldx, _ptr(Vt), ldvt,
                                           _ptr(Vt), ldvt, self.m, float(self.var), float(self.length_scale), _ptr(cov),
                                           ldvt, _stream()))
            return mean.cpu().numpy(), cov[:, :nt].cpu().numpy()
        return mean.cpu().numpy()
```

ital_amd/ital.py:

```python
import ctypes
import os

import numpy as np
import torch

from . import _lib, _mc_sampler, mvn_stream, sharding
from ._lib import ITAL_GENERIC_MAX_CALLS, ITAL_GENERIC_MAX_DIM, ITAL_GENERIC_MAX_REL, ITAL_MAX_T, ItalScoreDesc, check
from ._batch import (FUSED_LAUNCH_MAX as _FUSED_LAUNCH_MAX, LABEL_MODES as _LABEL_MODES, Scored, ensure_step_buffers,
                     fill_score_desc, fill_score_select, gp_model, lattice_label, lattice_tables, make_batch_buffers,
                     member_column, qmc_work, select_step)
from ._fast_round import FastRound
from ._generic_round import GenericRound
from ._mc_sampler import range_cuts as _range_cuts
from .gp import _ptr, _stream
from .retrieval_base import ActiveRetrievalBase, UnseenList

_FUSED_SELECT_MAX = _lib.ITAL_ROUND_MAX_CAND


class ITAL(ActiveRetrievalBase):

    def __init__(self, data=None, queries=[], length_scale=0.1, var=1.0, noise=1e-6, label_prob=1.0,
                 mistake_prob=0.0, top_candidates=None, change_estimation_subset=0, clip_cov=0,
                 label_estimation='mean', monte_carlo_num_rel=None, monte_carlo_num_fb=None, parallelized=True, *,
                 device=None, rank=0, world=1, group=None):
        ActiveRetrievalBase.__init__(self, data, queries, length_scale, var, noise, device=device, rank=rank,
                                     world=world, group=group)
        self.label_prob = label_prob
        self.mistake_prob = mistake_prob
        self.top_candidates = top_candidates
        self.change_estimation_subset = change_estimation_subset
        self.clip_cov = clip_cov
        self.label_estimation = label_estimation
        self.monte_carlo_num_rel = monte_carlo_num_rel
        self.monte_carlo_num_fb = monte_carlo_num_fb
        self.parallelized = parallelized
        self.eps = 1e-12
        self.last_scores = None
        self.keep_scores = False
        self.force_generic = False
        self._ce_subset = None
        self.qmc_work_bytes = int(os.environ.get("ITAL_QMC_WORK_BYTES", 1 << 30))
        self._last_batch = None
        self.pair_counter = None
        self.generic_pipeline = True
        self.event_pool = []
        self.profile = None
        self._fetch_bufs = None
        self.profile_steps = None
        self.round_call = True
        self._round_bufs = None
        self.last_round = None
        self._transport = None
        self._pinned = {}
        self.select_in_scorer = True
        self.mc_walk = [0, 0, 0.0]
        self.host_clock = None

    def _perfect_user(self):
        return self.label_prob >= 1 and self.mistake_prob <= 0

    def _fb_mode(self):
        return 0 if self._perfect_user() else (1 if self.label_prob >= 1 else 2)

    def _subset_mode(self):
        return self.change_estimation_subset is None or self.change_estimation_subset > 0

    def _mc_plan(self, nr, fb_mode):
        return _mc_sampler.mc_plan(nr, fb_mode, self.monte_carlo_num_rel, self.monte_carlo_num_fb)

    def _unsupported(self, k, n_unseen=0):
        if self.label_estimation not in _LABEL_MODES:
            return "label_estimation=%r" % (self.label_estimation,)
        if self.change_estimation_subset is None:
            if n_unseen > ITAL_GENERIC_MAX_DIM:
                return ("change_estimation_subset=None with %d candidates: orthants of that dimension (limit %d)"
                        % (n_unseen, ITAL_GENERIC_MAX_DIM))
            sub, max_dim = n_unseen, n_unseen
        else:
            sub = self.change_estimation_subset if self.change_estimation_subset > 0 else 0
            max_dim = sub + k
        if self._needs_generic():
            if max_dim > ITAL_GENERIC_MAX_DIM:
                return "orthant dimension %d (subset + batch) above %d" % (max_dim, ITAL_GENERIC_MAX_DIM)
            if k > ITAL_GENERIC_MAX_REL:
                return "batches larger than %d with the general scorer" % ITAL_GENERIC_MAX_REL
            fb_mode = self._fb_mode()
            for nr in range(1, k + 1):
                _, npat, _, nfb = self._mc_plan(nr, fb_mode)
                if npat * (2 + nfb) > ITAL_GENERIC_MAX_CALLS:
                    return ("%d orthant probabilities per candidate at greedy step %d: set monte_carlo_num_rel / "
                            "monte_carlo_num_fb (reference ital.py:293-297)" % (npat * (2 + nfb), nr))
        elif k > ITAL_MAX_T:
            return ("batches larger than %d with full enumeration: set monte_carlo_num_rel (reference ital.py:293-297)"
                    % ITAL_MAX_T)
        return None

    def _needs_generic(self):
        return (self._subset_mode() or not self._perfect_user() or self.force_generic or self._clip_active()
                or self.monte_carlo_num_rel is not None or self.monte_carlo_num_fb is not None)

    def _clip_active(self):
        return bool(self.clip_cov) and 0 < self.clip_cov < 1

    def _mark(self, stage=None, t=0, size=0, start=None):
        if self.profile is None:
            return None
        ev = self.event_pool.pop() if self.event_pool else torch.cuda.Event(enable_timing=True)
        ev.record()
        if start is not None:
            self.profile.append((stage, t, size, start, ev))
        return ev

    def _event(self):
        if self.event_pool:
            return self.event_pool.pop()
        ev = torch.cuda.Event(enable_timing=True)
        ev.record()
        return ev

    def _buffers(self, kmax):
        gp = self.gp
        b = self._fetch_bufs
        if b is not None and b["kmax"] >= kmax and b["ldw"] == gp.cap and b["gp"] is gp:
            return b
        b = make_batch_buffers(gp.device, kmax, gp.ldx, gp.cap, gp.ldv, gp.world)
        b["gp"] = gp
        self._fetch_bufs = b
        self._round_bufs = None
        return b

    def _start_afresh(self):
        ActiveRetrievalBase._start_afresh(self)
        if self._round_bufs is not None:
            self._round_bufs.drop_prepared()
            self._round_bufs.invalidate()
        self._fetch_bufs = None
        self._round_bufs = None
        self._ce_subset = None

    @property
    def _dev_list(self):
        return None if self._round_bufs is None else self._round_bufs.device_list

    def _candidate_list(self, candidates=None):
        if candidates is None:
            candidates = self._unseen_array()
        if self.change_estimation_subset is None:
            self._ce_subset = [int(i) for i in candidates]
        elif self.change_estimation_subset > 0:
            self._ce_subset = sorted(int(i) for i in np.random.choice(
                candidates, min(len(candidates), self.change_estimation_subset), replace=False))
        else:
            self._ce_subset = None
        if self.top_candidates is not None:
            top_candidates = self.top_candidates
            if isinstance(self.top_candidates, float):
                labelled = len(self.queries) + len(self.relevant_ids) + len(self.irrelevant_ids)
                top_candidates = min(len(candidates), int(self.top_candidates * labelled))
            if (top_candidates > 0) and (top_candidates < len(candidates)):
                top_ind = np.argpartition(self.rel_mean[candidates], -top_candidates)[-top_candidates:]
                candidates = candidates[top_ind]
        return candidates

    def fetch_unlabelled(self, k, show_progress=False):
        gp = self.gp
        if gp.m == 0:
            raise RuntimeError("fetch_unlabelled() needs a fitted relevance model: call update() first or pass queries "
                               "(the reference fails with an AttributeError at gp.py:222)")
        unseen = self._unseen_list()
        k = min(int(k), len(unseen))
        if k <= 0:
            return []
        why = self._unsupported(k, len(unseen))
        if why is not None:
            raise NotImplementedError("ital_amd device scorer: %s is not implemented" % why)
        if (self.top_candidates is None and not self._needs_generic() and self.round_call and self.select_in_scorer
                and self._round_possible(k, unseen)):
            self._ce_subset = None
            self._last_batch = None
            return self._select_round(k, unseen)
        candidates = self._candidate_list(unseen.array())
        if len(candidates) < k:
            if len(candidates) > 0:
                self._select(len(candidates), candidates)
            raise ValueError("attempt to get argmax of an empty sequence")
        return self._select(k, candidates)

    def _shard(self, candidates, b=None):
        gp = self.gp
        dev = gp.device
        cand = np.asarray(candidates, dtype=np.int64)
        if gp.world == 1:
            loc_rows, pos_offset, gpos = cand, 0, None
        else:
            loc_rows, pos_offset, gpos = sharding.shard_candidates(cand, gp.row0, gp.row1, self._ascending(candidates))
        n_loc = len(loc_rows)
        cand_d = torch.from_numpy((loc_rows - gp.row0).astype(np.int32)).to(dev) if n_loc else \
            torch.zeros(1, dtype=torch.int32, device=dev)
        gpos_d = torch.from_numpy(gpos).to(dev) if gpos is not None else None
        if b is not None:
            ensure_step_buffers(b, n_loc, 0, dev)
            alive = b["alive"]
            alive.fill_(1)
        else:
            alive = torch.ones(max(n_loc, 1), dtype=torch.uint8, device=dev)
        return cand, n_loc, pos_offset, cand_d, gpos_d, alive

    def _ascending(self, candidates):
        u = self.__dict__.get("_unseen")
        return u is not None and candidates is u[0]._flat

    def _qmc_workspace(self, b, t, n_loc):
        want = int(_lib.lib().ital_round_workspace(t, max(n_loc, 1), max(self.qmc_work_bytes // 8, 1 << 16)))
        return qmc_work(b, want, self.gp.device)

    def _sel_parts_doubles(self, k, n_loc):
        return int(_lib.lib().ital_sel_parts_len(k, n_loc, max(self.qmc_work_bytes // 8, 1 << 16)))

    def _select(self, k, candidates):
        self._last_batch = None
        generic = self._needs_generic()
        if not generic and self.round_call and self.select_in_scorer and self._round_possible(k, candidates):
            return self._select_round(k, candidates)
        if self._round_bufs is not None:
            self._round_bufs.invalidate()
        return self._fetch_generic(k, candidates) if generic else self._select_steps(k, candidates)

    def _user(self):
        return float(self.noise), float(self.eps), _LABEL_MODES[self.label_estimation]

    def _step_desc(self, b, scored, t, k, n_alive, tail, fused):
        gp = self.gp
        n_loc = scored.n
        desc = ItalScoreDesc()
        desc.t = t
        fill_score_desc(desc, gp, b, scored, self._user())
        if t >= 3:
            jump, jumppat, vk = lattice_tables(b, t, gp.device)
            desc.jump, desc.jumppat, desc.vk = _ptr(jump), _ptr(jumppat), _ptr(vk)
            for j in range(6):
                desc.seed[j] = mvn_stream.GLOBAL.state[j]
            work = self._qmc_workspace(b, t, n_loc)
            desc.work, desc.work_doubles = _ptr(work), work.numel()
            if self.profile is not None and n_loc > 0:
                k0, k1 = self._event(), self._event()
                desc.ev_start, desc.ev_stop = k0.cuda_event, k1.cuda_event
                self.profile.append((lattice_label(work, t, n_loc), t, n_alive if not gp.collective else n_loc, k0, k1))
        if tail:
            ensure_step_buffers(b, n_loc, self._sel_parts_doubles(k, n_loc), gp.device)
            fill_score_select(desc, gp, b, gp.m, b["ret"] if fused else None)
        return desc

    def _select_steps(self, k, candidates):
        gp = self.gp
        lib = _lib.lib()
        with torch.cuda.device(gp.device):
            b = self._buffers(k)
            st = _stream()
            cand, n_loc, pos_offset, cand_d, gpos_d, alive = self._shard(candidates, b)
            mi = b["mi"]
            scored = Scored(mi, cand_d, alive, n_loc, pos_offset, gpos_d, gp.row0)
            self.last_scores = []
            stream = mvn_stream.GLOBAL
            saved_stream = (stream.state, stream.draws)
            n_alive = len(candidates)
            b["ret"][b["kmax"]:].zero_()
            for t in range(1, k + 1):
                tail = self.select_in_scorer and 0 < n_loc <= _FUSED_SELECT_MAX
                fused = not gp.collective and 0 < n_loc <= (_FUSED_SELECT_MAX if tail else _FUSED_LAUNCH_MAX)
                desc = self._step_desc(b, scored, t, k, n_alive, tail, fused)
                ev0 = self._mark() if t < 3 else None
                check(lib.ital_score_step(ctypes.byref(desc), st))
                if t < 3:
                    self._mark("score", t, n_alive, ev0)
                if self.keep_scores:
                    self.last_scores.append(mi.clone())
                if not (tail and fused):
                    select_step(gp, b, scored, gp_model(gp), t - 1, st, fused=fused, local=not tail, mark=self._mark)
                if t < k:
                    ev0 = self._mark() if t == 1 else None
                    member_column(self, gp_model(gp), b, t - 1, st)
                    if t == 1:
                        self._mark("cross_cov", t, gp.m, ev0)
                stream.advance(mvn_stream.step_draws(t, n_alive))
                n_alive -= 1
            host = self._download(b["ret"], "the picks of the round", self._step_estimate_s(k, n_loc)).tolist()
            ret, status = host[:k], host[b["kmax"]]
            if status & 6:
                gp.status.bitwise_and_(~6)
                stream.state, stream.draws = saved_stream
                return self._fetch_generic(k, candidates)
        if status:
            gp.check_status(status)
        self._last_batch = (b, list(ret))
        return [int(i) for i in ret]

    def _round_possible(self, k, candidates):
        gp = self.gp
        n = len(candidates)
        if n < k:
            return False
        if not gp.collective:
            return n <= _FUSED_SELECT_MAX
        if not isinstance(candidates, UnseenList) or self._round_transport() is None:
            return False
        bounds = [sharding.row_range(gp.n_total, gp.world, r)[0] for r in range(gp.world)] + [gp.n_total]
        sizes = np.diff([candidates.count_below(x) for x in bounds])
        return bool(sizes.min() >= 1 and sizes.max() <= _FUSED_SELECT_MAX)

    @staticmethod
    def _step_estimate_s(k, n_loc):
        if k < 3:
            return 0.0
        prime = (31, 47, 73, 113, 173, 263, 397, 593, 907, 1361)[min(k - 1, 10) - 1]
        return float(n_loc) * (2 ** k) * 16 * prime * (k - 1) / 1e11

    def _download(self, tensor, what, step_estimate_s=0.0):
        gp = self.gp
        if not gp.collective:
            return tensor.cpu()
        kind = self._transport[1] if self._transport else None
        comm = kind[1] if kind and kind[0] == "nccl" else None
        if comm is None:
            e = sharding._RAW_COMMS.get((id(gp.group), str(gp.device)))
            comm = e[1] if e else None
        name = {"nccl": "raw_nccl", "host": "host"}[kind[0]] if kind else ("raw_nccl (per step)" if comm else "torch_dist")
        return sharding.await_download(tensor, what, gp.group, gp.device, comm, gp.rank, gp.world, name, pinned=self._pinned,
                                       step_estimate_s=step_estimate_s)

    def _round_transport(self):
        gp = self.gp
        cached = self._transport
        if cached is not None and cached[0] is gp.group:
            return cached[1]
        kind = None
        import torch.distributed as dist
        if gp.group is not None and dist.is_initialized():
            if dist.get_backend(gp.group) == "nccl":
                comm = sharding.raw_comm(gp.group, gp.device)
                kind = ("nccl", comm) if comm else None
            else:
                kind = ("host", None)
        if os.environ.get("ITAL_ROUND_TRANSPORT") == "none":
            kind = None
        elif os.environ.get("ITAL_ROUND_TRANSPORT") == "host" and kind is not None:
            kind = ("host", None)
        if kind is not None:
            self._transport = (gp.group, kind)
        return kind

    def _select_round(self, k, candidates):
        round_ = FastRound(self, k, candidates)
        with torch.cuda.device(self.gp.device):
            return round_.run()

    def _fetch_generic(self, k, candidates):
        self._last_batch = None
        with torch.cuda.device(self.gp.device):
            return GenericRound(self, k, candidates).run()
```

ital_amd/retrieval_base.py:

```python
import numpy as np

from . import tune
from .gp import GaussianProcess


class IdSet(set):

    _serial = 0

    def __init__(self, *a):
        set.__init__(self, *a)
        IdSet._serial += 1 << 20
        self.changes = IdSet._serial


def _counting(name):
    base = getattr(set, name)

    def method(self, *a, **kw):
        self.changes += 1
        return base(self, *a, **kw)
    method.__name__ = name
    method.__doc__ = base.__doc__
    return method


for _name in ("add", "discard", "remove", "pop", "clear", "update", "difference_update", "intersection_update",
              "symmetric_difference_update", "__ior__", "__iand__", "__isub__", "__ixor__"):
    setattr(IdSet, _name, _counting(_name))
del _name


class UnseenList(object):

    REBASE_AT = 4096

    def __init__(self, base):
        self.base = base
        self.removed = []
        self.version = 0
        self.last_removed = ()
        self._flat = base
        self._prev_flat = None

    def __len__(self):
        return len(self.base) - len(self.removed)

    def count_below(self, x):
        import bisect
        return int(np.searchsorted(self.base, x)) - bisect.bisect_left(self.removed, x)

    def remove(self, ids):
        import bisect
        ids = sorted(set(int(i) for i in ids))
        if not ids:
            return True
        arr = np.asarray(ids, dtype=np.int64)
        at = np.searchsorted(self.base, arr)
        if np.any(at >= len(self.base)) or np.any(self.base[np.minimum(at, len(self.base) - 1)] != arr):
            return False
        for i in ids:
            j = bisect.bisect_left(self.removed, i)
            if j < len(self.removed) and self.removed[j] == i:
                return False
        prev = self._flat
        for i in ids:
            bisect.insort(self.removed, i)
        self.version += 1
        self.last_removed = tuple(ids)
        self._flat, self._prev_flat = None, (prev, arr) if prev is not None else None
        return True

    def in_rows(self, row0, row1):
        import bisect
        a, b = int(np.searchsorted(self.base, row0)), int(np.searchsorted(self.base, row1))
        part = self.base[a:b]
        r0, r1 = bisect.bisect_left(self.removed, row0), bisect.bisect_left(self.removed, row1)
        if r1 > r0:
            part = np.delete(part, np.searchsorted(part, np.asarray(self.removed[r0:r1], dtype=np.int64)))
        return part

    def array(self):
        if self._flat is None:
            prev = self._prev_flat
            if prev is not None:
                self._flat = np.delete(prev[0], np.searchsorted(prev[0], prev[1]))
            else:
                self._flat = np.delete(self.base, np.searchsorted(self.base, np.asarray(self.removed, dtype=np.int64)))
            self._prev_flat = None
            if len(self.removed) >= self.REBASE_AT:
                self.base, self.removed = self._flat, []
        return self._flat


class ActiveRetrievalBase(object):

    gp_capacity = None

    def __init__(self, data=None, queries=[], length_scale=0.1, var=1.0, noise=1e-6, *, device=None, rank=0,
                 world=1, group=None):
        self.length_scale = length_scale
        self.var = var
        self.noise = noise
        self.device, self.rank, self.world, self.group = device, rank, world, group
        self.fit(data, queries)

    def fit(self, data, queries=[]):
        self.data = data
        self.queries = queries
        if self.data is not None:
            self.gp = GaussianProcess(self.data, self.length_scale, self.var, self.noise, device=self.device,
                                      rank=self.rank, world=self.world, group=self.group, capacity=self.gp_capacity)
            self.reset()
        else:
            self.gp = None

    def reset(self):
        self.rounds = 0
        self.relevant_ids = set()
        self.irrelevant_ids = set()
        self.unnameable_ids = set()
        self._last_batch = None
        self.gp.reset()
        if len(self.queries) > 0:
            n = len(self.data)
            self.gp.update_points(self.queries, [1] * len(self.queries), ind=list(range(n, n + len(self.queries))))
            self._fitted = True
        else:
            self._fitted = False

    def state_dict(self):
        from . import mvn_stream
        gp = self.gp
        return dict(version=1, n=len(self.data), hyper=(float(self.length_scale), float(self.var), float(self.noise)),
                    ind=[int(i) for i in gp.ind], y=(gp.y.copy() if gp.y is not None else np.zeros(0)),
                    appends=list(gp.appends), relevant_ids=sorted(self.relevant_ids),
                    irrelevant_ids=sorted(self.irrelevant_ids), unnameable_ids=sorted(self.unnameable_ids),
                    rounds=int(self.rounds), mvn_stream=(tuple(mvn_stream.GLOBAL.state), int(mvn_stream.GLOBAL.draws)),
                    np_random=np.random.get_state())

    def load_state_dict(self, sd, restore_stream=True):
        from . import mvn_stream
        if sd.get("version") != 1 or sd["n"] != len(self.data):
            raise ValueError("state_dict of another data set / version")
        if tuple(sd["hyper"]) != (float(self.length_scale), float(self.var), float(self.noise)):
            raise ValueError("state_dict was saved with other hyper-parameters: %r" % (sd["hyper"],))
        self.reset()
        at = self.gp.m
        ind, y = list(sd["ind"]), np.asarray(sd["y"], dtype=np.float64)
        for c in sd["appends"]:
            if c < 0:
                continue
            if c:
                self.gp.update(ind[at:at + c], y[at:at + c])
            at += c
        if self.gp.ind != ind:
            raise ValueError("state_dict does not match this learner's queries")
        self.relevant_ids = set(sd["relevant_ids"])
        self.irrelevant_ids = set(sd["irrelevant_ids"])
        self.unnameable_ids = set(sd["unnameable_ids"])
        self.rounds = int(sd["rounds"])
        self._fitted = self.gp.m > 0
        if restore_stream:
            mvn_stream.GLOBAL.state, mvn_stream.GLOBAL.draws = tuple(sd["mvn_stream"][0]), int(sd["mvn_stream"][1])
            if sd.get("np_random") is not None:
                np.random.set_state(sd["np_random"])
        return self

    @property
    def rel_mean(self):
        return self.gp.mean_host() if self._fitted else None

    def top_results(self, k=None):
        from ._lib import ITAL_TOPK_MAX
        if k is not None and self._fitted and 1 <= int(k) <= min(ITAL_TOPK_MAX, len(self.data)):
            return self.gp.topk_mean(int(k))
        ind = np.argsort(self.rel_mean, kind="stable")[::-1]
        return ind[:k] if k is not None else ind

    def get_unseen(self):
        return self._unseen_array().tolist()

    def _set_ids(self, name, value):
        self.__dict__[name] = value if isinstance(value, IdSet) else IdSet(value)
        self.__dict__["_unseen"] = None

    def _get_ids(self, name):
        try:
            return self.__dict__[name]
        except KeyError:
            raise AttributeError(name[1:]) from None

    relevant_ids = property(lambda self: self._get_ids("_relevant_ids"), lambda self, v: self._set_ids("_relevant_ids", v))
    irrelevant_ids = property(lambda self: self._get_ids("_irrelevant_ids"), lambda self, v: self._set_ids("_irrelevant_ids", v))
    unnameable_ids = property(lambda self: self._get_ids("_unnameable_ids"), lambda self, v: self._set_ids("_unnameable_ids", v))

    def _id_sizes(self):
        sets = (self.relevant_ids, self.irrelevant_ids, self.unnameable_ids)
        return tuple(len(q) for q in sets) + tuple(getattr(q, "changes", -1) for q in sets)

    def _unseen_list(self):
        u = self.__dict__.get("_unseen")
        if u is not None and u[1] == self._id_sizes():
            return u[0]
        seen = self.relevant_ids | self.irrelevant_ids | self.unnameable_ids
        if not seen:
            arr = np.arange(len(self.data), dtype=np.int64)
        else:
            mask = np.ones(len(self.data), dtype=bool)
            mask[np.fromiter(seen, dtype=np.int64, count=len(seen))] = False
            arr = np.flatnonzero(mask)
        lst = UnseenList(arr)
        self.__dict__["_unseen"] = (lst, self._id_sizes())
        return lst

    def _unseen_array(self):
        return self._unseen_list().array()

    def _unseen_after(self, new_ids, sizes_before):
        u = self.__dict__.get("_unseen")
        if u is None or u[1] != sizes_before:
            self.__dict__["_unseen"] = None
            return
        ids = set(int(i) for i in new_ids)
        if not u[0].remove(ids):
            self.__dict__["_unseen"] = None
            return
        self.__dict__["_unseen"] = (u[0], self._id_sizes())

    def fetch_unlabelled(self, k):
        raise NotImplementedError('fetch_unlabelled() has to be implemented in a derived class.')

    def update(self, feedback):
        rel, irr, unnameable = self.partition_feedback(feedback)
        sizes_before = self._id_sizes()
        if len(rel) + len(irr) > 0:
            self.gp.update(rel + irr, np.concatenate((np.ones(len(rel)), -1 * np.ones(len(irr)))),
                           row_cache=self._batch_rows())
            self._fitted = True
            self.relevant_ids.update(rel)
            self.irrelevant_ids.update(irr)
            self.rounds += 1
        new_unnameable = [i for i in unnameable if i not in self.unnameable_ids]
        self.unnameable_ids.update(unnameable)
        self._unseen_after(rel + irr + new_unnameable, sizes_before)

    def revoke(self, ids):
        ids = list(dict.fromkeys(int(i) for i in ids))
        for i in ids:
            if not (i in self.relevant_ids or i in self.irrelevant_ids or i in self.unnameable_ids):
                raise ValueError("sample %d never got feedback" % i)
        labelled = [i for i in ids if i in self.relevant_ids or i in self.irrelevant_ids]
        if labelled:
            self.gp.remove(labelled)
        for i in ids:
            self.relevant_ids.discard(i)
            self.irrelevant_ids.discard(i)
            self.unnameable_ids.discard(i)
        self.__dict__["_unseen"] = None
        self._fitted = self.gp.m > 0

    def _start_afresh(self):
        self.__dict__["_unseen"] = None
        self._last_batch = None

    def add_data(self, rows):
        rows = np.asarray(rows, dtype=np.float64)
        if rows.size == 0:
            return self
        if rows.ndim != 2 or rows.shape[1] != np.shape(self.data)[1]:
            raise ValueError("rows must be a k-by-%d array" % np.shape(self.data)[1])
        if self.world > 1:
            raise NotImplementedError("row sharding cannot grow yet: add_data() needs all rows on one rank")
        self.gp.extend(rows)
        self.data = self.gp.X_host
        self._start_afresh()
        return self

    def set_params(self, length_scale=None, var=None, noise=None):
        self.gp.set_params(length_scale, var, noise)
        self.length_scale, self.var, self.noise = self.gp.length_scale, self.gp.var, self.gp.noise
        self._start_afresh()
        return self

    def tune_params(self, grid=tune.default_grids['ls_only'], criterion='lml', apply=True, verbose=0):
        best, score = tune.optimize_session_params(self, grid, criterion=criterion, verbose=verbose)
        if score == -np.inf:
            raise np.linalg.LinAlgError("no candidate of the grid has a positive definite kernel matrix of the labelled samples")
        if apply:
            self.set_params(**best)
        return best, score

    def relabel(self, feedback):
        changed = []
        for i, fb in feedback.items():
            old = 1 if i in self.relevant_ids else -1 if i in self.irrelevant_ids else 0 if i in self.unnameable_ids else None
            new = 1 if fb > 0 else -1 if fb < 0 else 0
            if old is not None and old != new:
                changed.append(i)
        if changed:
            self.revoke(changed)
        self.update(feedback)

    def _batch_rows(self):
        last = getattr(self, "_last_batch", None)
        if not last:
            return None
        b, picks = last
        return b["XB"], {int(i): slot for slot, i in enumerate(picks)}

    def updated_prediction(self, feedback, test_ind, cov_mode='full'):
        rel, irr, _ = self.partition_feedback(feedback)
        if len(rel) + len(irr) == 0:
            return self.gp.predict_stored(test_ind, cov_mode=cov_mode)
        rel.sort()
        irr.sort()
        return self.gp.updated_prediction(rel + irr, np.concatenate((np.ones(len(rel)), -1 * np.ones(len(irr)))),
                                          test_ind, cov_mode=cov_mode)

    def partition_feedback(self, feedback):
        rel, irr, unnameable = [], [], []
        for i, fb in feedback.items():
            if fb > 0:
                if i in self.irrelevant_ids:
                    raise RuntimeError('Cannot change feedback once given.')
                elif i not in self.relevant_ids:
                    rel.append(i)
            elif fb < 0:
                if i in self.relevant_ids:
                    raise RuntimeError('Cannot change feedback once given.')
                elif i not in self.irrelevant_ids:
                    irr.append(i)
            else:
                unnameable.append(i)
        return rel, irr, unnameable
```

Baseline: 15.92 million candidates/s.

## Speculatively prepare GP append and next candidate list inside the fetch round

At the end of each fetch round, the device now speculatively runs the label-independent part of the Cholesky append (the new L rows and whitening) for the picked samples. It also compacts the next round's candidate list and writes the picks into a pinned host buffer signalled by an event. When the following update() matches the speculation, only a small commit kernel runs: it solves for the new alpha entries and updates mu and s2. Otherwise the full append and list-compaction paths are used. This aims to take append latency and the host download sync off the critical path, at the cost of extra state tracking, invalidation hooks and wasted work when the speculation misses.

```diff
diff --git a/include/ital_hip.h b/include/ital_hip.h
--- a/include/ital_hip.h
+++ b/include/ital_hip.h
@@ -64,8 +64,12 @@
     double* mu;
     double* s2;
     int* status;
+    int* pd_flag;
 } ital_append_desc;
 int ital_gp_append(const ital_append_desc* a, hipStream_t stream);
+
+int ital_gp_append_prepare(const ital_append_desc* a, hipStream_t stream);
+int ital_gp_append_commit(const ital_append_desc* a, hipStream_t stream);
 
 int ital_whiten_append(const double* X, const double* xnorm, int64_t n, int ldx, const double* Xnew,
                        const double* snew, int c, const double* L21, int ldw, const double* L22,
@@ -176,8 +180,14 @@
     void* nccl_comm;
     int (*exchange)(void* ctx, const double* record, double* records_all, int rec_len, hipStream_t stream);
     void* exchange_ctx;
+    int64_t* host_ret;
+    void* ret_event;
+    const ital_append_desc* spec_append;
+    int32_t* cand_next;
 } ital_round_desc;
 int ital_fetch_round(const ital_round_desc* r, hipStream_t stream);
+
+int ital_round_wait(void* ret_event);
 
 int ital_select_local(const double* mi, const int32_t* cand, const uint8_t* alive, int64_t n_cand, int64_t pos_offset,
                       const int64_t* gpos, int64_t row_offset, int rank, int mode, const double* mu, const double* s2,
diff --git a/ital_amd/_fast_round.py b/ital_amd/_fast_round.py
--- a/ital_amd/_fast_round.py
+++ b/ital_amd/_fast_round.py
@@ -5,7 +5,7 @@
 import numpy as np
 import torch
 
-from . import _lib, mvn_stream, sharding
+from . import _lib, _speculation, mvn_stream, sharding
 from ._batch import (Scored, ensure_step_buffers, fill_score_desc, fill_score_select, lattice_label, lattice_tables)
 from ._lib import check
 from .gp import _ptr, _stream
@@ -13,7 +13,7 @@
 
 PREPARED, COMPACT, UPLOAD = "prepared", "compact", "upload"
 
-DeviceList = collections.namedtuple("DeviceList", "buffers unseen version picks n_loc")
+DeviceList = collections.namedtuple("DeviceList", "buffers unseen version picks n_loc spec", defaults=(None,))
 
 
 class Prepared(collections.namedtuple("Prepared", "desc slot k n n_loc m begin cur state_before state_after draws events sig")):
@@ -50,6 +50,14 @@
         self.exchange_cb = None
         self.exchange_exc = None
         self.device_list = None
+        self.landing = None
+
+    def landing_buffer(self):
+        if self.landing is None:
+            ev = torch.cuda.Event()
+            ev.record()
+            self.landing = (torch.empty(self.b["kmax"] + 1, dtype=torch.int64, pin_memory=True), ev)
+        return self.landing
 
     def invalidate(self):
         self.device_list = None
@@ -147,6 +155,8 @@
         self.listed = isinstance(candidates, UnseenList)
         self.stream = mvn_stream.GLOBAL
         self.lo = self.n_loc = self.rb = self.p = self.keep = self.t_call = None
+        self.follows = False
+        self.spec = (False, None)
 
     def run(self):
         L = self.L
@@ -155,6 +165,7 @@
         self.p = p = self._descriptor()
         L.last_round = (p.begin, p.slot)
         self._keep_scores()
+        self._speculate()
         saved_stream = (self.stream.state, self.stream.draws)
         self._stamp_call()
         self._call()
@@ -184,9 +195,13 @@
         plan = plan_round(self.candidates, rb, dl, p, L.keep_scores, k, n, gp.m, self.stream.state,
                           rb.signature(k) if p is not None else None)
         rb.invalidate()
+        self.follows = plan != UPLOAD
+        done = _speculation.list_verdict(dl.spec if dl is not None else None, self.follows, rb.cur ^ 1, n_loc) == _speculation.USE
         if plan == PREPARED:
             rb.next = None
             rb.cur = p.cur
+            if done:
+                p.desc.begin = 0
             return p.patch_share(n_loc, self.lo) if gp.collective else p
         rb.drop_prepared()
         if plan == COMPACT:
@@ -197,12 +212,31 @@
             c = self.candidates
             share = c.in_rows(gp.row0, gp.row1) if self.listed else np.asarray(c, dtype=np.int64)
             rb.lists[rb.cur][:n_loc].copy_(torch.from_numpy((share - gp.row0).astype(np.int32)))
-        return rb.prepare(0, k, n, gp.m, begin, rb.cur, self.stream.state, n_prev=n_prev, n_loc=n_loc, pos_offset=self.lo)
+        fresh = rb.prepare(0, k, n, gp.m, begin, rb.cur, self.stream.state, n_prev=n_prev, n_loc=n_loc, pos_offset=self.lo)
+        if plan == COMPACT and done:
+            fresh.desc.begin = 0
+        return fresh
 
     def _keep_scores(self):
         if self.L.keep_scores:
             self.keep = torch.zeros((self.k, self.n_loc), dtype=torch.float64, device=self.gp.device)
             self.p.desc.mi_keep = _ptr(self.keep)
+
+    def _speculate(self):
+        L, gp, rb, d = self.L, self.gp, self.rb, self.p.desc
+        d.host_ret = d.ret_event = d.spec_append = d.cand_next = None
+        app, lst = _speculation.may_speculate(getattr(gp, "speculate", False), self.follows, gp.collective, L.keep_scores,
+                                              self.k, self.n_loc, gp.m, gp.cap)
+        app = app and getattr(gp, "speculate_append", True)
+        if not (app or lst):
+            return
+        host, ev = rb.landing_buffer()
+        d.host_ret, d.ret_event = host.data_ptr(), ev.cuda_event
+        if app:
+            d.spec_append = ctypes.addressof(gp.speculative_append(rb.b["XB"], self.k))
+        if lst:
+            d.cand_next = _ptr(rb.lists[rb.cur ^ 1])
+        self.spec = (app, _speculation.ListSpec(rb.cur ^ 1, self.n_loc - self.k) if lst else None)
 
     def _stamp_call(self):
         hc = self.L.host_clock
@@ -231,7 +265,12 @@
         L, k, hc = self.L, self.k, self.L.host_clock
         if hc is not None:
             hc["enqueue_s"] += time.perf_counter() - self.t_call
-        host = L._download(self.rb.b["ret"], "the picks of the round", L._step_estimate_s(k, self.n_loc)).tolist()
+        if self.p.desc.host_ret:
+            host, ev = self.rb.landing_buffer()
+            check(_lib.lib().ital_round_wait(ev.cuda_event))
+            host = host.tolist()
+        else:
+            host = L._download(self.rb.b["ret"], "the picks of the round", L._step_estimate_s(k, self.n_loc)).tolist()
         if hc is not None:
             hc["t_download"] = time.perf_counter()
         keep = self.keep
@@ -242,14 +281,17 @@
         L, gp, c = self.L, self.gp, self.candidates
         if status & 8:
             raise RuntimeError("ital_amd: the candidate list kept on the device lost track of the host's (internal error)")
+        app, lst = self.spec
         if status & 6:
-            gp.status.bitwise_and_(~6)
+            gp.status.bitwise_and_(~(6 | (8 if lst else 0)))
             self.stream.state, self.stream.draws = saved_stream
             return L._fetch_generic(self.k, c.array() if self.listed else c)
         if status:
             gp.check_status(status)
         ret = [int(i) for i in ret]
         L._last_batch = (self.rb.b, list(ret))
+        if app:
+            gp.publish_speculation(ret, self.rb.b["XB"])
         if self.listed:
-            self.rb.device_list = DeviceList(self.rb, c, c.version, ret, self.n_loc)
+            self.rb.device_list = DeviceList(self.rb, c, c.version, ret, self.n_loc, lst)
         return ret
diff --git a/ital_amd/_lib.py b/ital_amd/_lib.py
--- a/ital_amd/_lib.py
+++ b/ital_amd/_lib.py
@@ -30,7 +30,7 @@
     _fields_ = [("rows", c_void_p), ("ldx", c_int), ("lb", ItalLabelBatch), ("X", c_void_p), ("xnorm", c_void_p), ("n", c_int64),
                 ("XT", c_void_p), ("XTn", c_void_p), ("L", c_void_p), ("ldl", c_int), ("alpha", c_void_p), ("ybuf", c_void_p),
                 ("V", c_void_p), ("ldv", c_int64), ("m", c_int), ("var", c_double), ("length_scale", c_double),
-                ("noise", c_double), ("mu", c_void_p), ("s2", c_void_p), ("status", c_void_p)]
+                ("noise", c_double), ("mu", c_void_p), ("s2", c_void_p), ("status", c_void_p), ("pd_flag", c_void_p)]
 
 
 class ItalScoreDesc(ctypes.Structure):
@@ -54,7 +54,8 @@
                 ("ev_stop", c_void_p * (ITAL_MAX_T + 1)), ("n_rows", c_int64), ("var", c_double), ("length_scale", c_double),
                 ("mi_keep", c_void_p), ("begin", c_int), ("cand_prev", c_void_p), ("n_prev", c_int64),
                 ("world", c_int), ("records_all", c_void_p), ("nccl_comm", c_void_p), ("exchange", EXCHANGE_FN),
-                ("exchange_ctx", c_void_p)]
+                ("exchange_ctx", c_void_p), ("host_ret", c_void_p), ("ret_event", c_void_p), ("spec_append", c_void_p),
+                ("cand_next", c_void_p)]
 
 
 class ItalGscoreDesc(ctypes.Structure):
@@ -111,6 +112,9 @@
                                    c_void_p, c_void_p]),
     "ital_stage_labelled": (c_int, [c_void_p, c_int, ItalLabelBatch, c_void_p, c_void_p, c_void_p, c_void_p]),
     "ital_gp_append": (c_int, [ctypes.POINTER(ItalAppendDesc), c_void_p]),
+    "ital_gp_append_prepare": (c_int, [ctypes.POINTER(ItalAppendDesc), c_void_p]),
+    "ital_gp_append_commit": (c_int, [ctypes.POINTER(ItalAppendDesc), c_void_p]),
+    "ital_round_wait": (c_int, [c_void_p]),
     "ital_predict": (c_int, [c_void_p, c_int64, c_int, c_void_p, c_void_p, c_int, c_void_p, c_int, c_void_p,
                              c_double, c_double, c_void_p, c_void_p, c_void_p, c_void_p, c_int64, c_int, c_void_p]),
     "ital_topk": (c_int, [c_void_p, c_int64, c_int64, c_int, c_void_p, c_void_p, c_void_p, c_void_p]),
diff --git a/ital_amd/_speculation.py b/ital_amd/_speculation.py
--- /dev/null
+++ b/ital_amd/_speculation.py
@@ -0,0 +1,34 @@
+import collections
+import os
+
+COMMIT, DISCARD = "commit", "discard"
+USE, FALL_BACK = "use", "fall back"
+
+Pending = collections.namedtuple("Pending", "ids m buffers rows params")
+
+ListSpec = collections.namedtuple("ListSpec", "cur n")
+
+
+def enabled():
+    return os.environ.get("ITAL_SPECULATE", "1") != "0"
+
+
+def may_speculate(on, follows, collective, keep_scores, k, n, m, cap):
+    if not on or not follows or collective or keep_scores:
+        return False, False
+    return (1 <= k <= 16 and m + k <= cap), n - k >= 1
+
+
+def append_verdict(pending, ids, m, buffers, rows, params, cap, collective=False):
+    if pending is None or collective:
+        return DISCARD
+    c = len(ids)
+    same = (tuple(int(i) for i in ids) == tuple(pending.ids) and m == pending.m and buffers == pending.buffers
+            and rows == pending.rows and tuple(params) == tuple(pending.params))
+    return COMMIT if same and 1 <= c <= 16 and m + c <= cap else DISCARD
+
+
+def list_verdict(spec, follows, cur, n):
+    if spec is None or not follows:
+        return FALL_BACK
+    return USE if (spec.cur, spec.n) == (cur, n) else FALL_BACK
diff --git a/ital_amd/csrc/chol.hip b/ital_amd/csrc/chol.hip
--- a/ital_amd/csrc/chol.hip
+++ b/ital_amd/csrc/chol.hip
@@ -1,5 +1,6 @@
 #include <hip/hip_runtime.h>
 #include <stdint.h>
+#include <stdio.h>
 
 #include "device_math.h"
 #include "ital_hip.h"
@@ -19,11 +20,12 @@
     double* y_w;
 };
 
-__global__ __launch_bounds__(1024) void chol_append_kernel(const double* XT, const double* XTn,
-                                                           int ldx, double* __restrict__ L, int ldl,
-                                                           double* __restrict__ alpha, const double* ynew,
-                                                           int m, int c, double var, double s, double noise,
-                                                           int* __restrict__ status, StageArgs sa) {
+template <bool PREP>
+__device__ __forceinline__ void chol_append_body(const double* XT, const double* XTn,
+                                                 int ldx, double* __restrict__ L, int ldl,
+                                                 double* __restrict__ alpha, const double* ynew,
+                                                 int m, int c, double var, double s, double noise,
+                                                 int* __restrict__ status, const StageArgs& sa) {
     __shared__ double S[16][17];
     __shared__ double tvec[16];
     __shared__ double Lb[64][65];
@@ -42,7 +44,10 @@
                 acc += v * v;
             }
             acc = wave_sum(acc);
-            if (lane == 0) { sa.XTn_w[j] = acc; sa.y_w[j] = sa.lb.y[j]; }
+            if (lane == 0) {
+                sa.XTn_w[j] = acc;
+                if (!PREP) sa.y_w[j] = sa.lb.y[j];
+            }
         }
         __threadfence_block();
         __syncthreads();
@@ -136,10 +141,12 @@
             acc = wave_sum(acc);
             if (lane == 0) S[j][q] = Lg[m + q] - acc;
         }
-        double acc = 0;
-        for (int r = lane; r < m; r += 64) acc += Lg[r] * alpha[r];
-        acc = wave_sum(acc);
-        if (lane == 0) tvec[j] = ynew[j] - acc;
+        if (!PREP) {
+            double acc = 0;
+            for (int r = lane; r < m; r += 64) acc += Lg[r] * alpha[r];
+            acc = wave_sum(acc);
+            if (lane == 0) tvec[j] = ynew[j] - acc;
+        }
     }
     CHOL_STAMP(3);
     __syncthreads();
@@ -165,6 +172,12 @@
             __builtin_amdgcn_wave_barrier();
             __builtin_amdgcn_fence(__ATOMIC_ACQUIRE, "workgroup");
         }
+        if (PREP) {
+            if (mine)
+                for (int b = 0; b < c; b++) L[(int64_t)(m + lane) * ldl + m + b] = b <= lane ? S[lane][b] : 0.0;
+            if (lane == 0) *status = bad ? 1 : 0;
+            return;
+        }
         double tv = mine ? tvec[lane] : 0.0;
         const double dd = mine ? S[lane][lane] : 1.0;
         for (int q = 0; q < c; q++) {
@@ -180,12 +193,96 @@
     }
 #ifdef ITAL_CHOL_TIMING
     CHOL_STAMP(4);
-    if (threadIdx.x == 0)
+    if (!PREP && threadIdx.x == 0)
         for (int i = 0; i < 4; i++) alpha[ldl - 8 + i] = (double)(tstamp[i + 1] - tstamp[i]);
 #endif
 }
 
-}
+__global__ __launch_bounds__(1024) void chol_append_kernel(const double* XT, const double* XTn,
+                                                           int ldx, double* __restrict__ L, int ldl,
+                                                           double* __restrict__ alpha, const double* ynew,
+                                                           int m, int c, double var, double s, double noise,
+                                                           int* __restrict__ status, StageArgs sa) {
+    chol_append_body<false>(XT, XTn, ldx, L, ldl, alpha, ynew, m, c, var, s, noise, status, sa);
+}
+
+__global__ __launch_bounds__(1024) void chol_prepare_kernel(const double* XT, const double* XTn, int ldx,
+                                                            double* __restrict__ L, int ldl, int m, int c, double var,
+                                                            double s, double noise, int* __restrict__ side, StageArgs sa) {
+    chol_append_body<true>(XT, XTn, ldx, L, ldl, nullptr, nullptr, m, c, var, s, noise, side, sa);
+}
+
+struct CommitArgs {
+    const double* L;
+    int ldl;
+    double* alpha;
+    double* ybuf;
+    ital_label_batch lb;
+    int m, c;
+    const double* V;
+    int64_t ldv, n;
+    double* mu;
+    double* s2;
+    int* status;
+    const int* side;
+};
+
+__global__ __launch_bounds__(256) void append_commit_kernel(CommitArgs a) {
+    __shared__ double tvec[16];
+    __shared__ double anew[16];
+    const int lane = threadIdx.x & 63, wave = threadIdx.x >> 6;
+    const int m = a.m, c = a.c;
+    for (int j = wave; j < c; j += 4) {
+        const double* Lg = a.L + (int64_t)(m + j) * a.ldl;
+        double acc = 0;
+        for (int r = lane; r < m; r += 64) acc += Lg[r] * a.alpha[r];
+        acc = wave_sum(acc);
+        if (lane == 0) tvec[j] = a.lb.y[j] - acc;
+    }
+    __syncthreads();
+    if (wave == 0) {
+        const bool mine = lane < c;
+        const double* Ll = a.L + (int64_t)(m + (mine ? lane : 0)) * a.ldl + m;
+        double tv = mine ? tvec[lane] : 0.0;
+        const double dd = mine ? Ll[lane] : 1.0;
+        for (int q = 0; q < c; q++) {
+            const double xq = readlane_f64(tv, q) / readlane_f64(dd, q);
+            if (lane == q) tv = xq;
+            else if (mine && lane > q) tv -= Ll[q] * xq;
+        }
+        if (mine) {
+            anew[lane] = tv;
+            if (blockIdx.x == 0) {
+                a.alpha[m + lane] = tv;
+                a.ybuf[lane] = a.lb.y[lane];
+            }
+        }
+        if (blockIdx.x == 0 && lane == 0) {
+            const int bad = *a.side;
+            if (bad) atomicOr(a.status, bad);
+        }
+    }
+    __syncthreads();
+    const int64_t i = (int64_t)blockIdx.x * blockDim.x + threadIdx.x;
+    if (i >= a.n) return;
+    double dvar = 0, dmu = 0;
+#pragma unroll
+    for (int j = 0; j < 16; j++) {
+        if (j < c) {
+            const double vn = a.V[(int64_t)(m + j) * a.ldv + i];
+            dvar += vn * vn;
+            dmu += vn * anew[j];
+        }
+    }
+    a.s2[i] -= dvar;
+    a.mu[i] += dmu;
+}
+
+}
+
+int ital_whiten_prepare(const double* X, const double* xnorm, int64_t n, int ldx, const double* Xnew, const double* snew, int c,
+                        const double* L21, int ldw, const double* L22, double* V, int64_t ldv, int m, double var,
+                        double length_scale, hipStream_t stream);
 
 extern "C" int ital_chol_append(const double* XT, const double* XTn, int ldx, double* L, int ldl, double* alpha,
                                 const double* ynew, int m, int c, double var, double length_scale, double noise,
@@ -212,3 +309,39 @@
     return ital_whiten_append(a->X, a->xnorm, a->n, a->ldx, a->XT + (int64_t)m * a->ldx, a->XTn + m, c, L21, a->ldl, L21 + m,
                               a->alpha + m, a->V, a->ldv, m, a->var, a->length_scale, a->mu, a->s2, stream);
 }
+
+static int append_desc_ok(const ital_append_desc* a, const char* who, bool split) {
+    static thread_local char msg[160];
+    const char* why = nullptr;
+    if (!a) why = "null descriptor";
+    else if (a->lb.c < 1 || a->lb.c > 16) why = "1..16 samples per call";
+    else if (a->m < 0 || a->m + a->lb.c > a->ldl) why = "factor capacity exceeded";
+    else if (a->ldx % 16 != 0) why = "ldx must be a multiple of 16";
+    else if (split && !a->pd_flag) why = "pd_flag (the side slot of the verdict) missing";
+    if (!why) return 0;
+    snprintf(msg, sizeof(msg), "%s: %s", who, why);
+    return ital_fail(-22, msg);
+}
+
+extern "C" int ital_gp_append_prepare(const ital_append_desc* a, hipStream_t stream) {
+    int rc = append_desc_ok(a, "ital_gp_append_prepare", true);
+    if (rc) return rc;
+    const int c = a->lb.c, m = a->m;
+    ital::StageArgs sa = {a->rows, a->lb, a->XT + (int64_t)m * a->ldx, a->XTn + m, nullptr};
+    ITAL_LAUNCH(ital::chol_prepare_kernel, dim3(1), dim3(1024), 0, stream, a->XT, a->XTn, a->ldx, a->L, a->ldl, m, c, a->var,
+                -2.0 * a->length_scale * a->length_scale, a->noise, a->pd_flag, sa);
+    if ((rc = ital_check_launch("ital_gp_append_prepare(chol)"))) return rc;
+    const double* L21 = a->L + (int64_t)m * a->ldl;
+    return ital_whiten_prepare(a->X, a->xnorm, a->n, a->ldx, a->XT + (int64_t)m * a->ldx, a->XTn + m, c, L21, a->ldl, L21 + m,
+                               a->V, a->ldv, m, a->var, a->length_scale, stream);
+}
+
+extern "C" int ital_gp_append_commit(const ital_append_desc* a, hipStream_t stream) {
+    const int rc = append_desc_ok(a, "ital_gp_append_commit", true);
+    if (rc) return rc;
+    ital::CommitArgs ca = {a->L, a->ldl, a->alpha, a->ybuf, a->lb, a->m, a->lb.c, a->V, a->ldv, a->n, a->mu, a->s2, a->status,
+                           a->pd_flag};
+    const int64_t blocks = a->n > 0 ? (a->n + 255) / 256 : 1;
+    ITAL_LAUNCH(ital::append_commit_kernel, dim3((unsigned)blocks), dim3(256), 0, stream, ca);
+    return ital_check_launch("ital_gp_append_commit");
+}
diff --git a/ital_amd/csrc/rbf.hip b/ital_amd/csrc/rbf.hip
--- a/ital_amd/csrc/rbf.hip
+++ b/ital_amd/csrc/rbf.hip
@@ -57,6 +57,7 @@
 #endif
 constexpr int KU = ITAL_KCOLS_KU;
 
+template <bool VONLY = false>
 __device__ __forceinline__ void kcols_body(const KcolsArgs& a) {
     __shared__ double tile[4][16][17];
     const int lane = threadIdx.x & 63;
@@ -146,19 +147,24 @@
 #pragma unroll
                 for (int q = 0; q < j; q++) acc -= a.L22[j * a.ldw + q] * vn[q];
                 vn[j] = acc / a.L22[j * a.ldw + j];
-                dvar += vn[j] * vn[j];
-                dmu += vn[j] * a.alpha_new[j];
+                if (!VONLY) {
+                    dvar += vn[j] * vn[j];
+                    dmu += vn[j] * a.alpha_new[j];
+                }
                 a.Vw[(int64_t)(a.m + j) * a.ldv + irow] = vn[j];
             } else {
                 vn[j] = 0;
             }
         }
-        a.s2[irow] -= dvar;
-        a.mu[irow] += dmu;
+        if (!VONLY) {
+            a.s2[irow] -= dvar;
+            a.mu[irow] += dmu;
+        }
     }
 }
 
 __global__ __launch_bounds__(256) void kcols_kernel(KcolsArgs a) { kcols_body(a); }
+__global__ __launch_bounds__(256) void kcols_prepare_kernel(KcolsArgs a) { kcols_body<true>(a); }
 
 __global__ __launch_bounds__(256) void kcols_seed_kernel(KcolsArgs a, SeedArgs s, unsigned nk) {
     if (blockIdx.x >= nk) {
@@ -273,6 +279,20 @@
     a.var = var; a.s = -2.0 * length_scale * length_scale; a.mode = MODE_WHITEN;
     a.L22 = L22; a.alpha_new = alpha_new; a.mu = mu; a.s2 = s2;
     return launch_kcols(a, stream, "ital_whiten_append");
+}
+
+int ital_whiten_prepare(const double* X, const double* xnorm, int64_t n, int ldx, const double* Xnew, const double* snew, int c,
+                        const double* L21, int ldw, const double* L22, double* V, int64_t ldv, int m, double var,
+                        double length_scale, hipStream_t stream) {
+    KcolsArgs a = {};
+    a.X = X; a.xnorm = xnorm; a.n = n; a.ldx = ldx; a.Xs = Xnew; a.sn = snew; a.c = c;
+    a.W = L21; a.ldw = ldw; a.V = V; a.Vw = V; a.ldv = ldv; a.m = m;
+    a.var = var; a.s = -2.0 * length_scale * length_scale; a.mode = MODE_WHITEN;
+    a.L22 = L22;
+    if (a.n <= 0) return 0;
+    if (a.m < 0 || (a.m > 0 && (!a.W || !a.V))) return ital_fail(-22, "ital_gp_append_prepare: W/V missing");
+    ITAL_LAUNCH(kcols_prepare_kernel, dim3((unsigned)((a.n + 63) / 64)), dim3(256), 0, stream, a);
+    return ital_check_launch("ital_gp_append_prepare(whiten)");
 }
 
 extern "C" int ital_predict(const double* Xt, int64_t nt, int ldx, const double* XT, const double* XTn, int m,
diff --git a/ital_amd/csrc/round.hip b/ital_amd/csrc/round.hip
--- a/ital_amd/csrc/round.hip
+++ b/ital_amd/csrc/round.hip
@@ -128,6 +128,34 @@
 
 using namespace ital;
 
+static int list_upkeep(int mode, const int32_t* cand_prev, int64_t n_prev, int32_t* cand_new, int64_t n, const ital_score_desc& tpl,
+                       hipStream_t stream) {
+    uint8_t* alive = const_cast<uint8_t*>(tpl.alive);
+    if (mode == 1 && n_prev >= COMPACT_FROM) {
+        const unsigned ntiles = (unsigned)((n_prev + COMPACT_TILE - 1) / COMPACT_TILE);
+        if (!tpl.sel_parts || tpl.sel_parts_len * 2 < (int64_t)ntiles + 1)
+            return ital_fail(-22, "ital_fetch_round: step.sel_parts too small for the tile counts of the list upkeep (ital_sel_parts_len)");
+        int* counts = reinterpret_cast<int*>(tpl.sel_parts);
+        ITAL_LAUNCH(compact_count_kernel, dim3(ntiles), dim3(1024), 0, stream, alive, n_prev, counts);
+        ITAL_LAUNCH(compact_scatter_kernel, dim3(ntiles), dim3(1024), 0, stream, cand_prev, alive, n_prev, cand_new, counts);
+        ITAL_LAUNCH(compact_rearm_kernel, dim3(ntiles), dim3(1024), 0, stream, alive, n, tpl.sel_ret, tpl.batch.kmax,
+                    tpl.status, counts, (int)ntiles);
+        return ital_check_launch("ital_fetch_round(begin, tiles)");
+    }
+    ITAL_LAUNCH(fetch_begin_kernel, dim3(1), dim3(1024), 0, stream, mode, cand_prev, n_prev, cand_new, alive, n, tpl.sel_ret,
+                tpl.batch.kmax, tpl.status);
+    return ital_check_launch("ital_fetch_round(begin)");
+}
+
+extern "C" int ital_round_wait(void* ret_event) {
+    if (!ret_event) return ital_fail(-22, "ital_round_wait: null event");
+    if (hipEventSynchronize(static_cast<hipEvent_t>(ret_event)) != hipSuccess) {
+        (void)hipGetLastError();
+        return ital_fail(-5, "ital_round_wait: waiting for the round's event failed");
+    }
+    return 0;
+}
+
 extern "C" int ital_fetch_round(const ital_round_desc* r, hipStream_t stream) {
     if (!r) return ital_fail(-22, "ital_fetch_round: null descriptor");
     const ital_score_desc& tpl = r->step;
@@ -140,26 +168,18 @@
     if (tpl.n_cand > ITAL_ROUND_MAX_CAND) return ital_fail(-22, "ital_fetch_round: more than ITAL_ROUND_MAX_CAND candidates (use the per-step entry points)");
     if (!tpl.sel_record || !tpl.sel_ret) return ital_fail(-22, "ital_fetch_round: the round selects inside the scorer: sel_* missing");
     if (r->begin < 0 || r->begin > 2) return ital_fail(-22, "ital_fetch_round: begin must be 0, 1 or 2");
+    const bool after = r->host_ret || r->ret_event || r->spec_append || r->cand_next;
+    if (after && ranks) return ital_fail(-22, "ital_fetch_round: host_ret / spec_append / cand_next are for one rank (world == 0)");
+    if (after && (!r->host_ret || !r->ret_event))
+        return ital_fail(-22, "ital_fetch_round: spec_append / cand_next need host_ret and ret_event (the picks leave first)");
+    if (r->cand_next && (r->cand_next == tpl.cand || tpl.n_cand - r->k < 1))
+        return ital_fail(-22, "ital_fetch_round: cand_next must be a buffer of its own for at least one survivor");
+    if (r->spec_append && (r->spec_append->lb.c < r->k || r->spec_append->lb.c > tpl.batch.kmax || r->spec_append->rows != tpl.batch.XB))
+        return ital_fail(-22, "ital_fetch_round: spec_append must describe k .. kmax rows of step.batch.XB");
     if (r->begin == 2 && (!r->cand_prev || r->n_prev < tpl.n_cand || r->n_prev > ITAL_ROUND_MAX_CAND || r->cand_prev == tpl.cand))
         return ital_fail(-22, "ital_fetch_round: begin = 2 needs the previous list in a buffer of its own");
-    if (r->begin == 2 && r->n_prev >= COMPACT_FROM) {
-        const unsigned ntiles = (unsigned)((r->n_prev + COMPACT_TILE - 1) / COMPACT_TILE);
-        if (!tpl.sel_parts || tpl.sel_parts_len * 2 < (int64_t)ntiles + 1)
-            return ital_fail(-22, "ital_fetch_round: step.sel_parts too small for the tile counts of the list upkeep (ital_sel_parts_len)");
-        int* counts = reinterpret_cast<int*>(tpl.sel_parts);
-        uint8_t* alive = const_cast<uint8_t*>(tpl.alive);
-        ITAL_LAUNCH(compact_count_kernel, dim3(ntiles), dim3(1024), 0, stream, alive, r->n_prev, counts);
-        ITAL_LAUNCH(compact_scatter_kernel, dim3(ntiles), dim3(1024), 0, stream, r->cand_prev, alive, r->n_prev,
-                    const_cast<int32_t*>(tpl.cand), counts);
-        ITAL_LAUNCH(compact_rearm_kernel, dim3(ntiles), dim3(1024), 0, stream, alive, tpl.n_cand, tpl.sel_ret, tpl.batch.kmax,
-                    tpl.status, counts, (int)ntiles);
-        const int rc = ital_check_launch("ital_fetch_round(begin, tiles)");
-        if (rc) return rc;
-    } else if (r->begin) {
-        ITAL_LAUNCH(fetch_begin_kernel, dim3(1), dim3(1024), 0, stream, r->begin - 1, r->cand_prev, r->n_prev,
-                    const_cast<int32_t*>(tpl.cand), const_cast<uint8_t*>(tpl.alive), tpl.n_cand, tpl.sel_ret, tpl.batch.kmax,
-                    tpl.status);
-        const int rc = ital_check_launch("ital_fetch_round(begin)");
+    if (r->begin == 1 || r->begin == 2) {
+        const int rc = list_upkeep(r->begin - 1, r->cand_prev, r->n_prev, const_cast<int32_t*>(tpl.cand), tpl.n_cand, tpl, stream);
         if (rc) return rc;
     }
     auto step_desc = [&](int t) {
@@ -212,6 +232,17 @@
             if (rc) return rc;
         }
     }
+    if (after) {
+        if (hipMemcpyAsync(r->host_ret, tpl.sel_ret, sizeof(int64_t) * (size_t)(tpl.batch.kmax + 1), hipMemcpyDeviceToHost, stream) !=
+                hipSuccess ||
+            hipEventRecord(static_cast<hipEvent_t>(r->ret_event), stream) != hipSuccess) {
+            (void)hipGetLastError();
+            return ital_fail(-5, "ital_fetch_round: the copy of the picks to the host could not be enqueued");
+        }
+        int rc = 0;
+        if (r->spec_append && (rc = ital_gp_append_prepare(r->spec_append, stream))) return rc;
+        if (r->cand_next && (rc = list_upkeep(1, tpl.cand, tpl.n_cand, r->cand_next, tpl.n_cand - r->k, tpl, stream))) return rc;
+    }
     return 0;
 }
 
diff --git a/ital_amd/gp.py b/ital_amd/gp.py
--- a/ital_amd/gp.py
+++ b/ital_amd/gp.py
@@ -5,7 +5,7 @@
 import numpy as np
 import torch
 
-from . import _lib, sharding
+from . import _lib, _speculation, sharding
 from ._lib import check
 
 
@@ -75,6 +75,10 @@
             self.xnorm = torch.empty(max(self.n, 1), dtype=torch.float64, device=self.device)
             check(self._lib.ital_row_norms(_ptr(self.Xd), self.n, self.ldx, _ptr(self.xnorm), _stream()))
             self.status = torch.zeros(1, dtype=torch.int32, device=self.device)
+            self.speculate = _speculation.enabled()
+            self.speculate_append = os.environ.get("ITAL_SPECULATE_APPEND", "1") != "0"
+            self._spec = None
+            self._spec_flag = torch.zeros(1, dtype=torch.int32, device=self.device)
             self._gather_bufs = {}
             if capacity is None:
                 capacity = int(min(256, max(64, (2 << 30) // (8 * self.ldv))))
@@ -91,11 +95,13 @@
         XT = torch.zeros((cap, self.ldx), dtype=torch.float64, device=dev)
         XTn = torch.zeros(cap, dtype=torch.float64, device=dev)
         if old:
-            V[:old] = self.V
-            L[:old, :old] = self.L
-            alpha[:old] = self.alpha
-            XT[:old] = self.XT
-            XTn[:old] = self.XTn
+            m = self.m
+            self._spec = None
+            V[:m] = self.V[:m]
+            L[:m, :m] = self.L[:m, :m]
+            alpha[:m] = self.alpha[:m]
+            XT[:m] = self.XT[:m]
+            XTn[:m] = self.XTn[:m]
         self.V, self.L, self.alpha, self.XT, self.XTn, self.cap = V, L, alpha, XT, XTn, cap
 
     @property
@@ -154,6 +160,7 @@
         return out[:, : len(b)].cpu().numpy()
 
     def reset(self):
+        self._spec = None
         self.ind = []
         self.y = None
         self.m = 0
@@ -177,9 +184,12 @@
             return self
         hc = getattr(self, "host_clock", None)
         t0 = time.perf_counter() if hc is not None else 0.0
+        pending, self._spec = self._spec, None
         if row_cache is not None and all(i in row_cache[1] for i in ind):
             if len(ind) <= 16:
-                self._append_staged(row_cache[0], [row_cache[1][i] for i in ind], y)
+                commit = _speculation.append_verdict(pending, ind, self.m, self._buffer_key(), row_cache[0].data_ptr(),
+                                                     self._params(), self.cap, self.collective) == _speculation.COMMIT
+                self._append_staged(row_cache[0], [row_cache[1][i] for i in ind], y, commit=commit)
             else:
                 slots = torch.as_tensor([row_cache[1][i] for i in ind], dtype=torch.int64, device=self.device)
                 self._append(row_cache[0].index_select(0, slots), y)
@@ -196,6 +206,7 @@
         return self
 
     def update_points(self, points, y, ind=None):
+        self._spec = None
         pts = np.atleast_2d(np.asarray(points, dtype=np.float64))
         y = np.asarray(y, dtype=np.float64).reshape(-1)
         rows = torch.zeros((len(pts), self.ldx), dtype=torch.float64, device=self.device)
@@ -236,30 +247,53 @@
             sharding.all_reduce_sum(out, self.group)
         return out
 
-    def _append_staged(self, matrix, slots, y):
-        c = len(slots)
-        if self.m + c > self.cap:
-            self._alloc(max(2 * self.cap, self.m + c))
+    def _buffer_key(self):
+        return (self.V.data_ptr(), self.mu.data_ptr(), self.L.data_ptr(), self.cap)
+
+    def _params(self):
+        return float(self.var), float(self.length_scale), float(self.noise)
+
+    def _staged_desc(self, name, matrix, slots):
         if getattr(self, "_ybuf", None) is None:
             self._ybuf = torch.empty(16, dtype=torch.float64, device=self.device)
-        d = getattr(self, "_append_desc", None)
-        key = (self.V.data_ptr(), self.mu.data_ptr(), self.cap)
+        d = getattr(self, name, None)
+        key = self._buffer_key()
         if d is None or d[0] != key:
             a = _lib.ItalAppendDesc()
             a.ldx, a.X, a.xnorm, a.n = self.ldx, _ptr(self.Xd), _ptr(self.xnorm), self.n
             a.XT, a.XTn, a.L, a.ldl, a.alpha, a.ybuf = _ptr(self.XT), _ptr(self.XTn), _ptr(self.L), self.cap, _ptr(self.alpha), \
                 _ptr(self._ybuf)
             a.V, a.ldv, a.mu, a.s2, a.status = _ptr(self.V), self.ldv, _ptr(self.mu), _ptr(self.s2), _ptr(self.status)
-            self._append_desc = d = (key, a)
+            a.pd_flag = _ptr(self._spec_flag)
+            d = (key, a)
+            setattr(self, name, d)
         a = d[1]
         a.rows, a.m = _ptr(matrix), self.m
-        a.var, a.length_scale, a.noise = float(self.var), float(self.length_scale), float(self.noise)
-        a.lb.c = c
+        a.var, a.length_scale, a.noise = self._params()
+        a.lb.c = len(slots)
+        for j, slot in enumerate(slots):
+            a.lb.slot[j] = int(slot)
+        return a
+
+    def _append_staged(self, matrix, slots, y, commit=False):
+        c = len(slots)
+        if self.m + c > self.cap:
+            self._alloc(max(2 * self.cap, self.m + c))
+        a = self._staged_desc("_append_desc", matrix, slots)
         for j in range(c):
-            a.lb.slot[j] = int(slots[j])
             a.lb.y[j] = float(y[j])
-        check(self._lib.ital_gp_append(ctypes.byref(a), _stream()))
+        fn = self._lib.ital_gp_append_commit if commit else self._lib.ital_gp_append
+        check(fn(ctypes.byref(a), _stream()))
         self.m += c
+
+    def speculative_append(self, matrix, k):
+        return self._staged_desc("_spec_desc", matrix, range(k))
+
+    def publish_speculation(self, ids, matrix):
+        self._spec = _speculation.Pending(tuple(int(i) for i in ids), self.m, self._buffer_key(), _ptr(matrix), self._params())
+
+    def drop_speculation(self):
+        self._spec = None
 
     def _append(self, rows, y):
         lib, st = self._lib, _stream()
@@ -283,6 +317,7 @@
             self.m += c
 
     def remove(self, ind):
+        self._spec = None
         ind = [int(i) for i in ind]
         if not ind:
             return self
@@ -325,6 +360,7 @@
         check(self._lib.ital_whiten_rows(ctypes.byref(r), _stream()))
 
     def extend(self, rows):
+        self._spec = None
         rows = np.asarray(rows, dtype=np.float64)
         if rows.size == 0:
             return self
@@ -352,13 +388,14 @@
             self.n_total += k
             self.row1 = self.row0 + n_new
             self.X_host = np.concatenate((self.X_host, rows))
-            self._append_desc = None
+            self._append_desc = self._spec_desc = None
             self._gather_bufs = {}
             self._whiten_rows(n_old, k)
             self._replicate_mean()
         return self
 
     def set_params(self, length_scale=None, var=None, noise=None):
+        self._spec = None
         ls = float(self.length_scale if length_scale is None else length_scale)
         var = float(self.var if var is None else var)
         noise = float(self.noise if noise is None else noise)
@@ -379,7 +416,7 @@
                                                _ptr(yd[c0:c0 + c]), c0, c, var, ls, noise, _ptr(status), st))
                 self.check_status(int(status.item()))
                 self.L, self.alpha = L, alpha
-                self._append_desc = None
+                self._append_desc = self._spec_desc = None
             self.length_scale, self.length_scale_sq, self.var, self.noise = ls, ls * ls, var, noise
             if self.m:
                 self._whiten_rows(0, self.n)
diff --git a/ital_amd/ital.py b/ital_amd/ital.py
--- a/ital_amd/ital.py
+++ b/ital_amd/ital.py
@@ -168,6 +168,7 @@
         if gp.m == 0:
             raise RuntimeError("fetch_unlabelled() needs a fitted relevance model: call update() first or pass queries "
                                "(the reference fails with an AttributeError at gp.py:222)")
+        gp.drop_speculation()
         unseen = self._unseen_list()
         k = min(int(k), len(unseen))
         if k <= 0:
diff --git a/ital_amd/retrieval_base.py b/ital_amd/retrieval_base.py
--- a/ital_amd/retrieval_base.py
+++ b/ital_amd/retrieval_base.py
@@ -246,6 +246,7 @@
         self._unseen_after(rel + irr + new_unnameable, sizes_before)
 
     def revoke(self, ids):
+        self.gp.drop_speculation()
         ids = list(dict.fromkeys(int(i) for i in ids))
         for i in ids:
             if not (i in self.relevant_ids or i in self.irrelevant_ids or i in self.unnameable_ids):
@@ -284,6 +285,7 @@
         return self
 
     def tune_params(self, grid=tune.default_grids['ls_only'], criterion='lml', apply=True, verbose=0):
+        self.gp.drop_speculation()
         best, score = tune.optimize_session_params(self, grid, criterion=criterion, verbose=verbose)
         if score == -np.inf:
             raise np.linalg.LinAlgError("no candidate of the grid has a positive definite kernel matrix of the labelled samples")
```

New measurement: 15.86 million candidates/s. No clear change (-0.3%).
